# mct10/Speech-Vecalign

Measured on AMD Instinct MI355X. Metric: aligned doc-pairs/sec, higher is better.
Workload: dtype bf16; 1 GPU; synthetic 4096x4096 d=1024 bf16 embeddings, 4 overlap layers/side, 10 alignment types, band 14, coarse-to-fine (max_size_full_dp=300), 1024 doc-pairs per GPU per step; pipeline=1, N=4096, M=4096, d=1024, overlaps=4, parallelism=dp1 (pairs sharded, no collective)

## Files before the change

### include/svx.h

```cpp
#ifndef SVX_H
#define SVX_H

#include <stdint.h>

#ifdef __cplusplus
extern "C" {
#endif

typedef struct svx_ctx svx_ctx;

enum svx_dtype { SVX_F32 = 0, SVX_F16 = 1, SVX_BF16 = 2 };

enum svx_status {
    SVX_OK = 0,
    SVX_ERR_ARG = 1,
    SVX_ERR_OVERLAPS = 2,
    SVX_ERR_HIP = 3,
    SVX_ERR_TRACEBACK = 4,
    SVX_ERR_NOMEM = 5,
    SVX_ERR_EXTEND = 6,
    SVX_ERR_PATH = 7,
    SVX_ERR_BP = 8
};

#define SVX_MAX_LEVELS 16
#define SVX_MAX_TYPES 128
#define SVX_MAX_DIM 2048

int svx_create(int device_id, svx_ctx **out);
int svx_destroy(svx_ctx *ctx);
int svx_set_stream(svx_ctx *ctx, void *hip_stream);
int svx_synchronize(svx_ctx *ctx);
const char *svx_last_error(const svx_ctx *ctx);
const char *svx_version(void);
int64_t svx_scratch_bytes(const svx_ctx *ctx);


int svx_dense_costs(svx_ctx *ctx, const float *vecs0, int k0, int s0, const float *vecs1, int k1, int s1, int d,
                    const float *norm0, const float *norm1, int offset0, int offset1, float *costs);

int svx_dense_dp(svx_ctx *ctx, const float *cost, int s0, int s1, float pen, double *csum, int32_t *bp);

int svx_score_path(svx_ctx *ctx, const int32_t *xx, const int32_t *yy, int64_t n, const float *norm1,
                   const float *norm2, const float *vecs1, int rows1, const float *vecs2, int rows2, int d, float *out);

int svx_sparse_costs(svx_ctx *ctx, const float *vecs0, int k0, int xsize, const float *vecs1, int k1, int ysize,
                     int d, const float *norms0, const float *norms1, const int32_t *path, int A,
                     const int32_t *types_host, int T, int width_over2, float *costs, int32_t *b_offset);

int svx_sparse_dp(svx_ctx *ctx, const float *costs, const int32_t *b_offset_in, int A, int B,
                  const int32_t *types_host, int T, double del_penalty, int x_in_size, int y_in_size,
                  double *csum, int32_t *xp, int32_t *yp, int32_t *b_offset_out);


int svx_make_norm1(svx_ctx *ctx, float *vecs, int64_t rows, int d);

int svx_downsample(svx_ctx *ctx, const float *vecs, int k, int n, int d, float *half);

int svx_compute_norms(svx_ctx *ctx, const float *vecs0, int k0, int n0, const float *vecs1, int k1, int n1, int d,
                      const int32_t *idx, int samples_per_overlap, float *norms0);

int svx_del_penalty(svx_ctx *ctx, const float *scores, int64_t n, double frac, double *del_penalty);

int svx_dense_traceback(svx_ctx *ctx, const int32_t *bp, int s0, int s1, int32_t *align, int32_t *count);

int svx_sparse_traceback(svx_ctx *ctx, const double *csum, const int32_t *xp, const int32_t *yp,
                         const int32_t *b_offset_out, int a_out, int B, int xsize, int ysize, int32_t *align,
                         double *scores, int32_t *count);

int svx_search_path(svx_ctx *ctx, const int32_t *align, const int32_t *n_align, int upsample, int size0,
                    int size1, int32_t *path, int32_t *path_len);

int svx_gather_rows(svx_ctx *ctx, const void *table, int64_t n_rows, int d, int dtype, const int32_t *idx, int64_t n_out,
                    void *out);


int svx_mt19937_choice(uint32_t *key, int32_t *pos, int64_t n, int64_t size, int32_t *out);

int64_t svx_norm_index_count(int n, int m, int k0, int k1, int max_size_full_dp, int num_samps_for_norm, int have_norms0,
                             int have_norms1);
int64_t svx_knob_index_count(int n, int m, int max_size_full_dp, int costs_sample_size);

int svx_draw_indices(uint32_t *key, int32_t *pos, int n, int m, int k0, int k1, int max_size_full_dp, int costs_sample_size,
                     int num_samps_for_norm, int have_norms0, int have_norms1, int32_t *norm_idx, int32_t *knob_idx);

int svx_candidate_table(const char *seg_path, const char *cat_path, const char *ignore_path, int max_overlaps, int32_t *table,
                        int cap_lines, int32_t *n_lines, int64_t *n_candidates, char *err, int err_cap);

int64_t svx_format_alignments(const int32_t *rows, const double *scores, int64_t n, char *out, int64_t cap);


#define SVX_MARGIN_RATIO 0
#define SVX_MARGIN_DISTANCE 1
#define SVX_MARGIN_ABSOLUTE 2

int svx_unit_rows(svx_ctx *ctx, const void *rows, int dtype, int64_t n, int d, void *out, int out_dtype);

int svx_knn_mean_sim(svx_ctx *ctx, const void *queries, int q_dtype, int64_t n, const void *db, int db_dtype,
                     int64_t n_db, int d, int k, float *mean_sim);

int svx_knn_topk_merge(svx_ctx *ctx, const void *queries, int q_dtype, int64_t n, const void *db, int db_dtype,
                       int64_t n_db, int d, int k, float *topk, int first, float *mean_sim);

int svx_knn_search(svx_ctx *ctx, const void *queries, int q_dtype, int64_t n, const void *db, int db_dtype,
                   int64_t n_db, int d, int k, int64_t id_base, float *sims, int64_t *ids, int first);

int svx_knn_search_groups(svx_ctx *ctx, const void *queries, int q_dtype, const void *db, int db_dtype, int d, int k,
                          const int64_t *q_off, const int64_t *db_off, int n_groups, float *sims, int64_t *ids);

int svx_margin_scores(svx_ctx *ctx, const void *x, const void *y, int dtype, int64_t n, int d, const float *mean_xy,
                      const float *mean_yx, int margin, float *scores);


int svx_knn_list_means(svx_ctx *ctx, const float *sims, int64_t n, int k, float *mean);

int svx_margin_candidates(svx_ctx *ctx, const float *sims, const int64_t *ids, int64_t n, int k, const float *mean_q,
                          const float *mean_db, int64_t n_db, int64_t id_base, int margin, float *scores, int64_t *best_id,
                          float *best_score);

int64_t svx_mine_greedy(const int64_t *order, int64_t n_cand, const int64_t *src, const int64_t *tgt, int64_t n_src,
                        int64_t n_tgt, int64_t *out);


typedef struct svx_align_params {
    int32_t dtype;
    int32_t d;
    int32_t n_types;
    int32_t types[2 * SVX_MAX_TYPES];
    int32_t width_over2;
    int32_t max_size_full_dp;
    int32_t costs_sample_size;
    int32_t num_samps_for_norm;
    double del_percentile_frac;
    int32_t search_mode;
    int32_t reserved0;
} svx_align_params;

#define SVX_SEARCH_COARSE_TO_FINE 0
#define SVX_SEARCH_STRAIGHT 1

typedef struct svx_pair {
    const void *vecs0, *vecs1;
    int32_t n, m, k0, k1;
    const int32_t *norm_idx;
    const int32_t *knob_idx;
    const float *norms0, *norms1;
    int32_t *align;
    double *scores;
    int32_t *info;
    double *del_pen;
} svx_pair;

int svx_num_levels(int n, int m, int max_size_full_dp);
int64_t svx_knob_count(int n_l, int m_l, int costs_sample_size);

int svx_align_batch(svx_ctx *ctx, const svx_align_params *params, const svx_pair *pairs, int n_pairs);

int svx_alignment_rows(svx_ctx *ctx, int dtype, int d, const svx_pair *pairs, int n_pairs, double max_score, int64_t cap,
                       void *x_rows, void *y_rows, void *x_unit, void *y_unit, int unit_dtype, int32_t *src, int64_t *count);

#define SVX_CONCAT_MAX 8
typedef struct svx_frames { const int32_t *src, *tgt; } svx_frames;
typedef struct svx_concat_params {
    double  max_score;
    int32_t max_num_align;
    int32_t sample_rate;
    double  max_sil, max_dur;
    int32_t both_sides;
    int32_t pad;
    int64_t min_frames;
} svx_concat_params;
int svx_concat_rows(svx_ctx *ctx, int dtype, int d, const svx_pair *pairs, const svx_frames *frames, int n_pairs,
                    const svx_concat_params *params, int64_t cap, void *x_rows, void *y_rows, void *x_unit, void *y_unit,
                    int unit_dtype, int32_t *meta, int64_t *counts);

typedef struct svx_level_view {
    int32_t size0, size1, k0, k1;
    int32_t n_types, band;
    int32_t path_len, n_align;
    const float *n0, *n1;
    const double *del_penalty;
    const int32_t *searchpath;
    const float *a_b_costs;
    const int32_t *b_offset;
    const double *a_b_csum;
    const uint8_t *a_b_bp;
    const int32_t *a_b_xp, *a_b_yp;
    const int32_t *new_b_offset;
    const int32_t *alignments;
    const double *alignment_scores;
    const float *costs_1to1;
    const int32_t *x_y_tb_diag;
    const float *v0_l0, *v1_l0;
    const float *knob_scores;
    int32_t n_knob, reserved;
} svx_level_view;
int svx_debug_level(svx_ctx *ctx, int pair, int level, svx_level_view *out);
int svx_copy_to_host(svx_ctx *ctx, void *dst_host, const void *src_device, int64_t bytes);

int svx_set_profiling(svx_ctx *ctx, int on);
int svx_set_pipeline(svx_ctx *ctx, int on);
int svx_flush(svx_ctx *ctx);
double svx_stage_ms(svx_ctx *ctx, const char *stage);
int svx_stage_launches(svx_ctx *ctx, const char *stage);

#ifdef __cplusplus
}
#endif
#endif
```

### speech-vecalign_amd/csrc/svx_api.hip

```cpp
#include <stdarg.h>
#include <stdio.h>
#include <stdlib.h>
#include <string.h>

#include <chrono>
#include <functional>
#include <memory>
#include <type_traits>
#include <vector>

#include "svx_common.h"

static char g_err[512] = "";

int svx_fail(svx_ctx* ctx, int code, const char* fmt, ...) {
    char* dst = ctx ? ctx->err : g_err;
    va_list ap;
    va_start(ap, fmt);
    vsnprintf(dst, 512, fmt, ap);
    va_end(ap);
    return code;
}

static const char* kStageNames[] = {"pyr0",       "pyrN",     "pyr_aux",      "knob_scoresN", "knob",      "dense_costs",
                                    "dense_dp",   "path",     "band_costs0",  "band_costsN",  "band_dp0",  "band_dpN",
                                    "traceback",  "setup",    "total",        "host_plan",    "host_launch", "knob_sort", "knob_scores0", "pyr1", "tiles",
                                    "traceback0", "path0"};
enum {
    S_PYR0 = 0, S_PYRN, S_PYR_AUX, S_KNOB_SCORES, S_KNOB, S_DENSE_COSTS, S_DENSE_DP, S_PATH, S_BAND_COSTS0, S_BAND_COSTSN,
    S_BAND_DP0, S_BAND_DPN, S_TRACEBACK, S_SETUP, S_TOTAL, S_HOST_PLAN, S_HOST_LAUNCH, S_KNOB_SORT, S_KNOB_SCORES0, S_PYR1, S_TILES,
    S_TRACEBACK0, S_PATH0, S_COUNT
};

struct StageRec {
    int stage;
    hipEvent_t a, b;
};

struct BatchParams {
    SvxTypes tfinal, t11;
    int W, B, dtype, d, nsamp, n_types;
    double frac;
    bool straight, tiles, packable;
};

struct HalfState {
    char* arena = nullptr;
    size_t arena_bytes = 0;
    SvxPairDev* pinned = nullptr;
    size_t pinned_cap = 0;
    std::vector<SvxPairDev> host;
    SvxPairDev* dpairs = nullptr;
    int n_pairs = 0;
    int maxL = 0, max_ksum = 0, max_kn = 0, max_ds0 = 0, max_ds1 = 0, max_n0 = 0, max_tnd = 0;
    int max_nblk[SVX_MAX_LEVELS] = {0}, max_A[SVX_MAX_LEVELS] = {0};
    bool any_L0 = false;
    size_t o_tickets = 0;
    size_t o_planes = 0, b_planes = 0;
    double b_pyr[SVX_MAX_LEVELS] = {0}, b_bc[SVX_MAX_LEVELS] = {0}, b_knobN = 0, b_knob0 = 0, dense_cells = 0;
    BatchParams bp;
    bool chain_pending = false;
    bool chain_done_valid = false;
    hipEvent_t front_done = nullptr, chain_done = nullptr, upload_done = nullptr;
    bool upload_valid = false;
};

struct svx_ctx_ext : svx_ctx {
    double ms[S_COUNT];
    int launches[S_COUNT];
    std::vector<StageRec> recs;
    std::vector<StageRec> pending;
    double acc_ms[S_COUNT];
    long long acc_launches[S_COUNT];
    int pipeline;
    HalfState half[2];
    int last_split;
    hipStream_t chain;
    bool chain_ready;
    std::vector<hipEvent_t> ev_pool;
    size_t ev_next;
    hipStream_t side;
    hipStream_t helper;
    hipEvent_t side_fork, side_join;
    bool side_ready;
    int last_ntypes, last_band;
};

static inline svx_ctx_ext* X(svx_ctx* c) { return static_cast<svx_ctx_ext*>(c); }

struct StageScope {
    svx_ctx_ext* c;
    StageRec r;
    bool on;
    StageScope(svx_ctx* ctx, int stage) : c(X(ctx)), on(ctx->profiling != 0) {
        r.stage = stage;
        if (on) {
            (void)hipEventCreate(&r.a);
            (void)hipEventCreate(&r.b);
            (void)hipEventRecord(r.a, c->stream);
        }
    }
    ~StageScope() {
        if (on) {
            (void)hipEventRecord(r.b, c->stream);
            c->recs.push_back(r);
        }
        c->launches[r.stage]++;
    }
};

static void drop_pending(svx_ctx_ext* c) {
    for (auto& r : c->pending) { (void)hipEventDestroy(r.a); (void)hipEventDestroy(r.b); }
    c->pending.clear();
}

extern "C" {

const char* svx_version(void) { return "svx 0.1 (gfx950)"; }

int svx_create(int device_id, svx_ctx** out) {
    if (!out) return svx_fail(nullptr, SVX_ERR_ARG, "svx_create: out is NULL");
    int ndev = 0;
    hipError_t e = hipGetDeviceCount(&ndev);
    if (e != hipSuccess || ndev <= 0)
        return svx_fail(nullptr, SVX_ERR_HIP, "svx_create: no HIP device (%s)", hipGetErrorString(e));
    if (device_id < 0 || device_id >= ndev) return svx_fail(nullptr, SVX_ERR_ARG, "svx_create: device %d of %d", device_id, ndev);
    e = hipSetDevice(device_id);
    if (e != hipSuccess) return svx_fail(nullptr, SVX_ERR_HIP, "hipSetDevice: %s", hipGetErrorString(e));
    svx_ctx_ext* c = new svx_ctx_ext();
    c->device = device_id;
    c->stream = nullptr;
    c->arena = nullptr;
    c->arena_bytes = 0;
    c->arena_used = 0;
    c->err[0] = 0;
    c->profiling = 0;
    c->rows_buf = nullptr;
    c->rows_bytes = 0;
    c->rows_turn = 0;
    for (int i = 0; i < 2; i++) { c->rows_pin[i] = nullptr; c->rows_pin_cap[i] = 0; c->rows_up[i] = nullptr; c->rows_up_valid[i] = 0; }
    for (int i = 0; i < S_COUNT; i++) { c->ms[i] = -1.0; c->launches[i] = 0; }
    c->pipeline = 0;
    c->last_split = 0;
    c->chain = nullptr;
    c->chain_ready = false;
    c->ev_next = 0;
    c->last_ntypes = 0;
    c->last_band = 0;
    c->side_ready = false;
    *out = c;
    return SVX_OK;
}

int svx_destroy(svx_ctx* ctx) {
    if (!ctx) return SVX_OK;
    svx_ctx_ext* c = X(ctx);
    (void)hipSetDevice(ctx->device);
    (void)svx_flush(ctx);
    (void)hipStreamSynchronize(ctx->stream);
    if (c->chain_ready) (void)hipStreamSynchronize(c->chain);
    if (ctx->arena) (void)hipFree(ctx->arena);
    svxl_alignrows_release(ctx);
    drop_pending(c);
    for (auto& r : c->recs) { (void)hipEventDestroy(r.a); (void)hipEventDestroy(r.b); }
    if (c->side_ready) {
        (void)hipStreamSynchronize(c->side);
        (void)hipStreamDestroy(c->side);
        (void)hipStreamSynchronize(c->helper);
        (void)hipStreamDestroy(c->helper);
        (void)hipEventDestroy(c->side_fork);
        (void)hipEventDestroy(c->side_join);
    }
    if (c->chain_ready) (void)hipStreamDestroy(c->chain);
    for (auto e : c->ev_pool) (void)hipEventDestroy(e);
    for (int h = 0; h < 2; h++) {
        HalfState& H = c->half[h];
        if (H.arena) (void)hipFree(H.arena);
        if (H.pinned) (void)hipHostFree(H.pinned);
        if (H.front_done) (void)hipEventDestroy(H.front_done);
        if (H.chain_done) (void)hipEventDestroy(H.chain_done);
        if (H.upload_done) (void)hipEventDestroy(H.upload_done);
    }
    delete c;
    return SVX_OK;
}

int svx_set_stream(svx_ctx* ctx, void* hip_stream) {
    if (!ctx) return SVX_ERR_ARG;
    ctx->stream = reinterpret_cast<hipStream_t>(hip_stream);
    return SVX_OK;
}

int svx_synchronize(svx_ctx* ctx) {
    if (!ctx) return SVX_ERR_ARG;
    int rc = svx_flush(ctx);
    if (rc) return rc;
    SVX_HIP(ctx, hipStreamSynchronize(ctx->stream));
    return SVX_OK;
}

const char* svx_last_error(const svx_ctx* ctx) { return ctx ? ctx->err : g_err; }

int64_t svx_scratch_bytes(const svx_ctx* ctx) {
    if (!ctx) return 0;
    const svx_ctx_ext* c = static_cast<const svx_ctx_ext*>(ctx);
    return (int64_t)(ctx->arena_bytes + c->half[0].arena_bytes + c->half[1].arena_bytes + ctx->rows_bytes);
}

int svx_set_pipeline(svx_ctx* ctx, int on) {
    if (!ctx || on < 0 || on > 1) return SVX_ERR_ARG;
    if (X(ctx)->pipeline != on) {
        int rc = svx_flush(ctx);
        if (rc) return rc;
    }
    X(ctx)->pipeline = on;
    return SVX_OK;
}

static void fold_pending(svx_ctx_ext* c) {
    if (c->pending.empty()) return;
    (void)svx_flush(c);
    (void)hipStreamSynchronize(c->stream);
    if (c->side_ready) { (void)hipStreamSynchronize(c->side); (void)hipStreamSynchronize(c->helper); }
    for (auto& r : c->pending) {
        float ms = 0.f;
        if (hipEventElapsedTime(&ms, r.a, r.b) == hipSuccess) { c->acc_ms[r.stage] += ms; }
        (void)hipEventDestroy(r.a);
        (void)hipEventDestroy(r.b);
    }
    c->pending.clear();
}

int svx_set_profiling(svx_ctx* ctx, int on) {
    if (!ctx) return SVX_ERR_ARG;
    svx_ctx_ext* c = X(ctx);
    drop_pending(c);
    ctx->profiling = on;
    if (on == 2)
        for (int i = 0; i < S_COUNT; i++) { c->acc_ms[i] = 0.0; c->acc_launches[i] = 0; }
    return SVX_OK;
}

static int stage_index(const char* name) {
    for (int i = 0; i < S_COUNT; i++)
        if (strcmp(name, kStageNames[i]) == 0) return i;
    return -1;
}

double svx_stage_ms(svx_ctx* ctx, const char* stage) {
    if (!ctx || !stage) return -1.0;
    int i = stage_index(stage);
    if (i < 0) return -1.0;
    if (ctx->profiling == 2) {
        fold_pending(X(ctx));
        return X(ctx)->acc_ms[i];
    }
    return X(ctx)->ms[i];
}

int svx_stage_launches(svx_ctx* ctx, const char* stage) {
    if (!ctx || !stage) return -1;
    int i = stage_index(stage);
    if (i < 0) return -1;
    if (ctx->profiling == 2) return (int)X(ctx)->acc_launches[i];
    return X(ctx)->launches[i];
}

}

static int arena_reserve(svx_ctx* ctx, size_t bytes) {
    if (bytes <= ctx->arena_bytes) return SVX_OK;
    SVX_HIP(ctx, hipStreamSynchronize(ctx->stream));
    if (ctx->arena) SVX_HIP(ctx, hipFree(ctx->arena));
    ctx->arena = nullptr;
    ctx->arena_bytes = 0;
    size_t want = bytes + bytes / 16 + (1 << 20);
    hipError_t e = hipMalloc(&ctx->arena, want);
    if (e != hipSuccess) return svx_fail(ctx, SVX_ERR_NOMEM, "scratch arena: hipMalloc(%zu) failed: %s", want, hipGetErrorString(e));
    ctx->arena_bytes = want;
    return SVX_OK;
}

struct Bump;
template <class T>
static inline void set_off(T*& p, Bump& b, size_t bytes);

struct Bump {
    size_t off = 0;
    size_t take(size_t bytes) {
        size_t o = off;
        off += (bytes + 255) & ~(size_t)255;
        return o;
    }
};

template <class T>
static inline void set_off(T*& p, Bump& b, size_t bytes) {
    p = reinterpret_cast<T*>(b.take(bytes) + 1);
}

static int make_types(svx_ctx* ctx, const int32_t* types, int T, SvxTypes* out) {
    if (T < 0 || T > SVX_MAX_TYPES) return svx_fail(ctx, SVX_ERR_ARG, "%d alignment types (max %d)", T, SVX_MAX_TYPES);
    out->n = T;
    out->maxstep = 1;
    for (int t = 0; t < T; t++) {
        int x = types[2 * t], y = types[2 * t + 1];
        if (x < 1 || y < 1 || x > 100 || y > 100) return svx_fail(ctx, SVX_ERR_ARG, "alignment type (%d,%d): sizes must be >= 1", x, y);
        out->x[t] = (int8_t)x;
        out->y[t] = (int8_t)y;
        if (x + y > out->maxstep) out->maxstep = x + y;
    }
    out->x[T] = 0; out->y[T] = 1;
    out->x[T + 1] = 1; out->y[T + 1] = 0;
    return SVX_OK;
}

static int check_dim(svx_ctx* ctx, int d) {
    if (d <= 0 || d % 8 != 0 || d > SVX_MAX_DIM)
        return svx_fail(ctx, SVX_ERR_ARG, "embedding dimension %d: must be a positive multiple of 8, at most %d", d, SVX_MAX_DIM);
    return SVX_OK;
}

#define NEED(ctx, cond, ...) \
    do { if (!(cond)) return svx_fail(ctx, SVX_ERR_ARG, __VA_ARGS__); } while (0)

extern "C" {

int svx_dense_costs(svx_ctx* ctx, const float* vecs0, int k0, int s0, const float* vecs1, int k1, int s1, int d,
                    const float* norm0, const float* norm1, int offset0, int offset1, float* costs) {
    NEED(ctx, ctx && vecs0 && vecs1 && norm0 && norm1 && costs, "svx_dense_costs: null argument");
    NEED(ctx, k0 > offset0 && k1 > offset1 && offset0 >= 0 && offset1 >= 0, "svx_dense_costs: offsets (%d,%d) outside %d/%d layers", offset0, offset1, k0, k1);
    int rc = check_dim(ctx, d);
    if (rc) return rc;
    return svxl_dense_costs(ctx, vecs0 + (size_t)offset0 * s0 * d, s0, vecs1 + (size_t)offset1 * s1 * d, s1, d,
                            norm0 + (size_t)offset0 * s0, norm1 + (size_t)offset1 * s1, offset0 + 1, offset1 + 1, costs);
}

int svx_dense_dp(svx_ctx* ctx, const float* cost, int s0, int s1, float pen, double* csum, int32_t* bp) {
    NEED(ctx, ctx && bp && (cost || s0 == 0 || s1 == 0), "svx_dense_dp: null argument");
    NEED(ctx, s0 >= 0 && s1 >= 0, "svx_dense_dp: negative size");
    return svxl_dense_dp(ctx, cost, s0, s1, pen, csum, bp);
}

int svx_score_path(svx_ctx* ctx, const int32_t* xx, const int32_t* yy, int64_t n, const float* norm1, const float* norm2,
                   const float* vecs1, int rows1, const float* vecs2, int rows2, int d, float* out) {
    NEED(ctx, ctx && xx && yy && norm1 && norm2 && vecs1 && vecs2 && out, "svx_score_path: null argument");
    NEED(ctx, rows1 > 0 && rows2 > 0, "svx_score_path: empty vecs");
    int rc = check_dim(ctx, d);
    if (rc) return rc;
    return svxl_score_path(ctx, xx, yy, n, norm1, norm2, vecs1, rows1, vecs2, rows2, d, out);
}

int svx_sparse_costs(svx_ctx* ctx, const float* vecs0, int k0, int xsize, const float* vecs1, int k1, int ysize, int d,
                     const float* norms0, const float* norms1, const int32_t* path, int A, const int32_t* types_host, int T,
                     int width_over2, float* costs, int32_t* b_offset) {
    NEED(ctx, ctx && vecs0 && vecs1 && norms0 && norms1 && path && b_offset && (costs || T == 0), "svx_sparse_costs: null argument");
    NEED(ctx, width_over2 >= 1 && A >= 0, "svx_sparse_costs: bad width/path length");
    int rc = check_dim(ctx, d);
    if (rc) return rc;
    SvxTypes ty;
    rc = make_types(ctx, types_host, T, &ty);
    if (rc) return rc;
    int mx = 0, my = 0;
    for (int t = 0; t < T; t++) { if (ty.x[t] > mx) mx = ty.x[t]; if (ty.y[t] > my) my = ty.y[t]; }
    if (mx > k0) return svx_fail(ctx, SVX_ERR_OVERLAPS, "%d x overlaps requrested (via alignment_types), but vecs0 only has %d", mx, k0);
    if (my > k1) return svx_fail(ctx, SVX_ERR_OVERLAPS, "%d y overlaps requrested (via alignment_types), but vecs1 only has %d", my, k1);
    rc = arena_reserve(ctx, 256);
    if (rc) return rc;
    int* status = reinterpret_cast<int*>(ctx->arena);
    SVX_HIP(ctx, hipMemsetAsync(status, 0, sizeof(int), ctx->stream));
    rc = svxl_band_costs(ctx, vecs0, k0, xsize, vecs1, k1, ysize, d, SVX_F32, nullptr, nullptr, norms0, norms1, path, A, ty,
                         width_over2, costs, b_offset, status);
    if (rc) return rc;
    int hs = 0;
    SVX_HIP(ctx, hipMemcpyAsync(&hs, status, sizeof(int), hipMemcpyDeviceToHost, ctx->stream));
    SVX_HIP(ctx, hipStreamSynchronize(ctx->stream));
    if (hs != 0) return svx_fail(ctx, hs, "search path is not a unit-step lattice path starting at (0,0)");
    return SVX_OK;
}

int svx_sparse_dp(svx_ctx* ctx, const float* costs, const int32_t* b_offset_in, int A, int B, const int32_t* types_host,
                  int T, double del_penalty, int x_in_size, int y_in_size, double* csum, int32_t* xp, int32_t* yp,
                  int32_t* b_offset_out) {
    NEED(ctx, ctx && b_offset_in && csum && xp && yp && b_offset_out && (costs || T == 0), "svx_sparse_dp: null argument");
    NEED(ctx, A >= 1 && B >= 1, "svx_sparse_dp: empty cost band");
    SvxTypes ty;
    int rc = make_types(ctx, types_host, T, &ty);
    if (rc) return rc;
    return svxl_sparse_dp(ctx, costs, b_offset_in, A, B, ty, del_penalty, x_in_size, y_in_size, csum, xp, yp, b_offset_out);
}

int svx_make_norm1(svx_ctx* ctx, float* vecs, int64_t rows, int d) {
    NEED(ctx, ctx && (vecs || rows == 0), "svx_make_norm1: null argument");
    int rc = check_dim(ctx, d);
    if (rc) return rc;
    return svxl_make_norm1(ctx, vecs, rows, d);
}

int svx_downsample(svx_ctx* ctx, const float* vecs, int k, int n, int d, float* half) {
    NEED(ctx, ctx && vecs && (half || n < 2), "svx_downsample: null argument");
    int rc = check_dim(ctx, d);
    if (rc) return rc;
    const int h = n / 2;
    if (h <= 0 || k <= 0) return SVX_OK;
    const int nblk = (h + SVX_PYR_SLOTS - 1) / SVX_PYR_SLOTS;
    Bump b;
    size_t o_part = b.take((size_t)k * nblk * d * sizeof(float));
    size_t o_mean = b.take((size_t)k * d * sizeof(float));
    rc = arena_reserve(ctx, b.off);
    if (rc) return rc;
    float* part = reinterpret_cast<float*>(ctx->arena + o_part);
    float* mean = reinterpret_cast<float*>(ctx->arena + o_mean);
    if ((rc = svxl_pairsum(ctx, vecs, k, n, d, half, part, nblk))) return rc;
    if ((rc = svxl_colmean_plain(ctx, part, k, nblk, d, h, mean))) return rc;
    return svxl_sub_mean(ctx, half, k, h, d, mean);
}

int svx_compute_norms(svx_ctx* ctx, const float* vecs0, int k0, int n0, const float* vecs1, int k1, int n1, int d,
                      const int32_t* idx, int samples_per_overlap, float* norms0) {
    NEED(ctx, ctx && vecs0 && vecs1 && idx && norms0, "svx_compute_norms: null argument");
    NEED(ctx, n1 > 0 && samples_per_overlap > 0 && k1 > 0, "svx_compute_norms: nothing to sample");
    int rc = check_dim(ctx, d);
    if (rc) return rc;
    rc = arena_reserve(ctx, (size_t)d * sizeof(float) + 256);
    if (rc) return rc;
    float* rbar = reinterpret_cast<float*>(ctx->arena);
    if ((rc = svxl_sample_mean_plain(ctx, vecs1, k1, n1, d, idx, samples_per_overlap, rbar))) return rc;
    return svxl_norms_from_rbar(ctx, vecs0, (int64_t)k0 * n0, d, rbar, norms0);
}

int svx_del_penalty(svx_ctx* ctx, const float* scores, int64_t n, double frac, double* del_penalty) {
    NEED(ctx, ctx && scores && del_penalty && n > 0, "svx_del_penalty: null/empty argument");
    return svxl_del_penalty(ctx, scores, n, frac, del_penalty);
}

int svx_dense_traceback(svx_ctx* ctx, const int32_t* bp, int s0, int s1, int32_t* align, int32_t* count) {
    NEED(ctx, ctx && bp && align && count, "svx_dense_traceback: null argument");
    return svxl_dense_traceback(ctx, bp, s0, s1, align, count);
}

int svx_sparse_traceback(svx_ctx* ctx, const double* csum, const int32_t* xp, const int32_t* yp, const int32_t* b_offset_out,
                         int a_out, int B, int xsize, int ysize, int32_t* align, double* scores, int32_t* count) {
    NEED(ctx, ctx && csum && xp && yp && b_offset_out && align && scores && count, "svx_sparse_traceback: null argument");
    return svxl_sparse_traceback(ctx, csum, xp, yp, b_offset_out, a_out, B, xsize, ysize, align, scores, count);
}

int svx_search_path(svx_ctx* ctx, const int32_t* align, const int32_t* n_align, int upsample, int size0, int size1,
                    int32_t* path, int32_t* path_len) {
    NEED(ctx, ctx && align && n_align && path && path_len, "svx_search_path: null argument");
    return svxl_search_path(ctx, align, n_align, upsample, size0, size1, path, size0 + size1 + 4, path_len);
}

int svx_gather_rows(svx_ctx* ctx, const void* table, int64_t n_rows, int d, int dtype, const int32_t* idx, int64_t n_out, void* out) {
    NEED(ctx, ctx && table && idx && out, "svx_gather_rows: null argument");
    NEED(ctx, dtype == SVX_F32 || dtype == SVX_F16 || dtype == SVX_BF16, "svx_gather_rows: unknown dtype %d", dtype);
    int rc = check_dim(ctx, d);
    if (rc) return rc;
    return svxl_gather_rows(ctx, table, n_rows, d * (dtype == SVX_F32 ? 4 : 2), dtype, idx, n_out, out);
}

}

__global__ void k_init_batch(const SvxPairDev* pairs) {
    const SvxPairDev& P = pairs[blockIdx.x];
    if (threadIdx.x != 0) return;
    *P.status = 0;
    for (int l = 0; l <= P.L; l++) {
        if (P.lev[l].n_align) *P.lev[l].n_align = 0;
        if (P.lev[l].path_len) *P.lev[l].path_len = 0;
    }
    if (P.straight) {
        int* r = P.lev[0].align;
        r[0] = 0; r[1] = P.lev[0].n[0]; r[2] = 0; r[3] = P.lev[0].n[1];
        *P.lev[0].n_align = 1;
    }
}

static inline int ceil_div(int a, int b) { return (a + b - 1) / b; }

extern "C" int svx_copy_to_host(svx_ctx* ctx, void* dst_host, const void* src_device, int64_t bytes) {
    NEED(ctx, ctx && (bytes == 0 || (dst_host && src_device)) && bytes >= 0, "svx_copy_to_host: bad argument");
    if (bytes == 0) return SVX_OK;
    SVX_HIP(ctx, hipSetDevice(ctx->device));
    SVX_HIP(ctx, hipMemcpyAsync(dst_host, src_device, (size_t)bytes, hipMemcpyDeviceToHost, ctx->stream));
    SVX_HIP(ctx, hipStreamSynchronize(ctx->stream));
    return SVX_OK;
}

extern "C" int svx_debug_level(svx_ctx* ctx, int pair, int level, svx_level_view* out) {
    NEED(ctx, ctx && out, "svx_debug_level: null argument");
    svx_ctx_ext* cx = X(ctx);
    const int total = cx->half[0].n_pairs + (cx->last_split > 0 ? cx->half[1].n_pairs : 0);
    NEED(ctx, pair >= 0 && pair < total, "svx_debug_level: pair %d of the last batch (%d pairs)", pair, total);
    const bool second = cx->last_split > 0 && pair >= cx->last_split;
    const SvxPairDev& P = second ? cx->half[1].host[pair - cx->last_split] : cx->half[0].host[pair];
    NEED(ctx, level >= 0 && level <= P.L, "svx_debug_level: level %d (the pair has %d)", level, P.L + 1);
    const SvxLevel& Lv = P.lev[level];
    memset(out, 0, sizeof(*out));
    out->size0 = Lv.n[0]; out->size1 = Lv.n[1];
    out->k0 = P.K[0]; out->k1 = P.K[1];
    out->n_types = level == 0 ? cx->last_ntypes : 1;
    out->band = cx->last_band;
    out->n0 = Lv.nrm[0]; out->n1 = Lv.nrm[1];
    out->del_penalty = Lv.pen;
    SVX_HIP(ctx, hipSetDevice(ctx->device));
    int rc = svx_synchronize(ctx);
    if (rc) return rc;
    if (Lv.n_align) SVX_HIP(ctx, hipMemcpy(&out->n_align, Lv.n_align, sizeof(int), hipMemcpyDeviceToHost));
    out->alignments = Lv.align;
    const bool refined = (level < P.L) || (P.L == 0);
    if (refined) {
        SVX_HIP(ctx, hipMemcpy(&out->path_len, Lv.path_len, sizeof(int), hipMemcpyDeviceToHost));
        out->searchpath = Lv.path;
        out->a_b_costs = Lv.costs;
        out->b_offset = Lv.boff;
        out->a_b_csum = Lv.csum;
        out->a_b_bp = Lv.bpk;
        out->a_b_xp = Lv.xp;
        out->a_b_yp = Lv.yp;
        out->new_b_offset = Lv.boff_out;
        out->alignment_scores = Lv.scores;
    }
    if (level == P.L && !P.straight) {
        out->costs_1to1 = P.dcost;
        out->x_y_tb_diag = P.dbp;
    }
    out->knob_scores = Lv.kscore;
    out->n_knob = Lv.kn;
    if (level >= 1) {
        out->v0_l0 = Lv.P[0];
        out->v1_l0 = Lv.P[1];
    }
    return SVX_OK;
}

static int plan_half(svx_ctx* ctx, HalfState& H, const BatchParams& bp, const svx_align_params* prm, const svx_pair* pairs, int n_pairs) {
    const int d = bp.d;
    const size_t esz = bp.dtype == SVX_F32 ? 4 : 2;
    const SvxTypes& tfinal = bp.tfinal;
    const int B = bp.B;
    const bool straight = bp.straight, tiles = bp.tiles, packable = bp.packable;
    int mx = 0, my = 0;
    for (int t = 0; t < tfinal.n; t++) { if (tfinal.x[t] > mx) mx = tfinal.x[t]; if (tfinal.y[t] > my) my = tfinal.y[t]; }
    std::vector<SvxPairDev>& host = H.host;
    host.assign(n_pairs, SvxPairDev());
    H.n_pairs = n_pairs;
    H.bp = bp;
    H.maxL = H.max_ksum = H.max_kn = H.max_ds0 = H.max_ds1 = H.max_n0 = H.max_tnd = 0;
    H.any_L0 = false;
    H.o_tickets = 0;
    H.o_planes = H.b_planes = 0;
    H.b_knobN = H.b_knob0 = H.dense_cells = 0;
    for (int l = 0; l < SVX_MAX_LEVELS; l++) { H.max_nblk[l] = H.max_A[l] = 0; H.b_pyr[l] = H.b_bc[l] = 0; }
    Bump bump;
    const size_t o_desc = bump.take((size_t)n_pairs * sizeof(SvxPairDev));
#define OFF(ptr_field, bytes) set_off(ptr_field, bump, bytes)
    for (int p = 0; p < n_pairs; p++) {
        const svx_pair& in = pairs[p];
        SvxPairDev& P = host[p];
        memset(&P, 0, sizeof(P));
        NEED(ctx, in.vecs0 && in.vecs1 && in.align && in.scores && in.info && in.knob_idx, "pair %d: null pointer", p);
        NEED(ctx, in.n >= 1 && in.m >= 1 && in.k0 >= 1 && in.k1 >= 1, "pair %d: empty document or no overlap layers", p);
        if (mx > in.k0) return svx_fail(ctx, SVX_ERR_OVERLAPS, "%d x overlaps requrested (via alignment_types), but vecs0 only has %d", mx, in.k0);
        if (my > in.k1) return svx_fail(ctx, SVX_ERR_OVERLAPS, "%d y overlaps requrested (via alignment_types), but vecs1 only has %d", my, in.k1);
        const int L = straight ? 0 : svx_num_levels(in.n, in.m, prm->max_size_full_dp);
        P.straight = straight ? 1 : 0;
        NEED(ctx, L < SVX_MAX_LEVELS, "pair %d: %d pyramid levels (max %d)", p, L + 1, SVX_MAX_LEVELS);
        P.v[0] = in.vecs0; P.v[1] = in.vecs1;
        P.K[0] = in.k0; P.K[1] = in.k1;
        P.L = L; P.d = d;
        P.norm_override[0] = in.norms0 != nullptr;
        P.norm_override[1] = in.norms1 != nullptr;
        P.status = in.info + 1;
        if (L > H.maxL) H.maxL = L;
        if (in.n > H.max_n0) H.max_n0 = in.n;
        if (L == 0) H.any_L0 = true;
        if (in.k0 + in.k1 > H.max_ksum) H.max_ksum = in.k0 + in.k1;
        const int S_from[2] = {in.k0 > 0 ? ceil_div(prm->num_samps_for_norm, in.k0) : 0,
                               in.k1 > 0 ? ceil_div(prm->num_samps_for_norm, in.k1) : 0};
        const int32_t* nidx = in.norm_idx;
        const int32_t* kidx = in.knob_idx;
        for (int l = 0; l <= L; l++) {
            SvxLevel& Lv = P.lev[l];
            const int K[2] = {in.k0, in.k1};
            for (int s = 0; s < 2; s++) {
                Lv.n[s] = (s == 0 ? in.n : in.m) >> l;
                Lv.nblk[s] = ceil_div((Lv.n[s] + 1) / 2, SVX_PYR_SLOTS);
                if (Lv.nblk[s] > H.max_nblk[l]) H.max_nblk[l] = Lv.nblk[s];
            }
            for (int s = 1; s >= 0; s--) {
                const bool skip = (l == 0) && P.norm_override[1 - s];
                Lv.S[s] = skip ? 0 : S_from[s];
                Lv.sidx[s] = nullptr;
                if (Lv.S[s] > 0) {
                    NEED(ctx, nidx != nullptr, "pair %d: norm_idx is NULL", p);
                    Lv.sidx[s] = nidx;
                    nidx += (size_t)K[s] * Lv.S[s];
                }
            }
            for (int s = 0; s < 2; s++) {
                if (l >= 1) {
                    Lv.npart[s] = P.lev[l - 1].nblk[s];
                    OFF(Lv.P[s], (size_t)(l == 1 ? 1 : K[s]) * Lv.n[s] * d * sizeof(float));
                    OFF(Lv.part[s], (size_t)K[s] * Lv.npart[s] * d * sizeof(float));
                    OFF(Lv.mean[s], (size_t)K[s] * d * sizeof(float));
                } else {
                    OFF(Lv.inv[s], (size_t)K[s] * Lv.n[s] * sizeof(float));
                }
                OFF(Lv.rbar[s], (size_t)d * sizeof(float));
                if (l == 0 && P.norm_override[s]) Lv.nrm[s] = const_cast<float*>(s == 0 ? in.norms0 : in.norms1);
                else OFF(Lv.nrm[s], (size_t)K[s] * Lv.n[s] * sizeof(float));
            }
            const int64_t kn = svx_knob_count(Lv.n[0], Lv.n[1], prm->costs_sample_size);
            Lv.kn = (int)kn;
            Lv.kx = kidx;
            Lv.ky = kidx + kn;
            kidx += 2 * kn;
            if (Lv.kn > H.max_kn) H.max_kn = Lv.kn;
            OFF(Lv.kscore, (size_t)kn * sizeof(float));
            OFF(Lv.korder, (size_t)kn * sizeof(int));
            OFF(Lv.kys, (size_t)kn * sizeof(int));
            OFF(Lv.kstart, (size_t)(Lv.n[0] + 1) * sizeof(int));
            if (in.del_pen) Lv.pen = in.del_pen + l;
            else OFF(Lv.pen, sizeof(double));
            const bool refined = (l < L) || (L == 0);
            const int rows_cap = Lv.n[0] + Lv.n[1] + 2;
            if (refined) {
                const int cap = Lv.n[0] + Lv.n[1] + 4;
                const int T = (l == 0) ? tfinal.n : 1;
                Lv.path_cap = cap;
                if (cap > H.max_A[l]) H.max_A[l] = cap;
                OFF(Lv.path, (size_t)cap * 2 * sizeof(int));
                OFF(Lv.path_len, sizeof(int));
                OFF(Lv.cstart, (size_t)(cap / 16 + 3) * sizeof(int));
                OFF(Lv.nchunks, sizeof(int));
                if (!tiles) OFF(Lv.costs, (size_t)(T > 0 ? T : 1) * cap * B * sizeof(float));
                OFF(Lv.boff, (size_t)cap * sizeof(int));
                OFF(Lv.csum, (size_t)(cap + 2) * B * sizeof(double));
                if (packable) {
                    OFF(Lv.bpk, (size_t)(cap + 2) * B);
                } else {
                    OFF(Lv.xp, (size_t)(cap + 2) * B * sizeof(int));
                    OFF(Lv.yp, (size_t)(cap + 2) * B * sizeof(int));
                }
                OFF(Lv.boff_out, (size_t)(cap + 2) * sizeof(int));
            }
            if (l == 0) {
                Lv.align = in.align;
                Lv.scores = in.scores;
                Lv.n_align = in.info;
            } else {
                OFF(Lv.align, (size_t)rows_cap * 4 * sizeof(int));
                OFF(Lv.scores, (size_t)rows_cap * sizeof(double));
                OFF(Lv.n_align, sizeof(int));
            }
            const double krows = (double)K[0] * Lv.n[0] + (double)K[1] * Lv.n[1], rows = (double)Lv.n[0] + Lv.n[1];
            if (l == 0) {
                H.b_pyr[0] += krows * d * esz;
                H.b_bc[0] += krows * d * esz;
                H.b_knob0 += (double)kn * d * esz;
            } else {
                if (l == 1) H.b_pyr[1] += ((double)K[0] * in.n + (double)K[1] * in.m) * d * esz + rows * d * 4.0;
                else H.b_pyr[l] += (krows + rows) * d * 4.0;
                H.b_pyr[l - 1] += l >= 2 ? krows * d * 4.0 : 0.0;
                if (l < L) { H.b_bc[l] += rows * d * 4.0; H.b_knobN += (double)kn * d * 4.0; }
            }
        }
        const SvxLevel& top = P.lev[L];
        if (!straight) {
            if (top.n[0] > H.max_ds0) H.max_ds0 = top.n[0];
            if (top.n[1] > H.max_ds1) H.max_ds1 = top.n[1];
            H.dense_cells += (double)top.n[0] * top.n[1];
            OFF(P.dcost, (size_t)top.n[0] * top.n[1] * sizeof(float));
            OFF(P.ddot, (size_t)top.n[0] * top.n[1] * sizeof(float));
            OFF(P.dbp, (size_t)(top.n[0] + top.n[1] + 1) * (top.n[0] + 1) * sizeof(int));
        }
        if (tiles) {
            const long long TI = in.n / 32 + 1, TJ = in.m / 32 + 1;
            P.t_nd = (int)(TI + TJ - 1);
            long long tcap = (long long)P.t_nd * ((B + 64) / 32 + 2);
            if (tcap > TI * TJ) tcap = TI * TJ;
            NEED(ctx, tcap < (1ll << 30), "pair %d: too many tiles", p);
            P.t_cap = (int)tcap;
            OFF(P.t_lo, (size_t)P.t_nd * sizeof(int));
            OFF(P.t_cnt, (size_t)P.t_nd * sizeof(int));
            OFF(P.t_pref, (size_t)(P.t_nd + 1) * sizeof(int));
            OFF(P.t_flag, (size_t)P.t_cap * sizeof(int));
        }
    }
#undef OFF
    for (int p = 0; p < n_pairs; p++)
        if (host[p].t_nd > H.max_tnd) H.max_tnd = host[p].t_nd;
    if (tiles) {
        H.o_tickets = bump.take(((size_t)(H.max_tnd + 2) * n_pairs + 2) * sizeof(int));
        H.b_planes = svxl_band_tiles_scratch(tfinal);
        if (H.b_planes) H.o_planes = bump.take(H.b_planes);
    }
    if (bump.off > H.arena_bytes) {
        SVX_HIP(ctx, hipDeviceSynchronize());
        if (H.arena) SVX_HIP(ctx, hipFree(H.arena));
        H.arena = nullptr;
        H.arena_bytes = 0;
        const size_t want = bump.off + bump.off / 16 + (1 << 20);
        hipError_t e = hipMalloc(&H.arena, want);
        if (e != hipSuccess) return svx_fail(ctx, SVX_ERR_NOMEM, "scratch arena: hipMalloc(%zu) failed: %s", want, hipGetErrorString(e));
        H.arena_bytes = want;
    }
    const size_t desc_bytes = (size_t)n_pairs * sizeof(SvxPairDev);
    if (desc_bytes > H.pinned_cap) {
        SVX_HIP(ctx, hipDeviceSynchronize());
        if (H.pinned) SVX_HIP(ctx, hipHostFree(H.pinned));
        H.pinned = nullptr;
        H.pinned_cap = 0;
        SVX_HIP(ctx, hipHostMalloc(reinterpret_cast<void**>(&H.pinned), desc_bytes + desc_bytes / 8, hipHostMallocDefault));
        H.pinned_cap = desc_bytes + desc_bytes / 8;
    }
    char* base = H.arena;
    const char* ulo = reinterpret_cast<const char*>(1);
    const char* uhi = reinterpret_cast<const char*>(bump.off + 1);
    auto patch = [&](auto& ptr) {
        const char* v = reinterpret_cast<const char*>(ptr);
        if (v >= ulo && v < uhi) ptr = reinterpret_cast<typename std::remove_reference<decltype(ptr)>::type>(base + (v - ulo));
    };
    for (int p = 0; p < n_pairs; p++) {
        SvxPairDev& P = host[p];
        const svx_pair& in = pairs[p];
        for (int l = 0; l <= P.L; l++) {
            SvxLevel& Lv = P.lev[l];
            for (int s = 0; s < 2; s++) {
                patch(Lv.P[s]); patch(Lv.part[s]); patch(Lv.mean[s]); patch(Lv.rbar[s]); patch(Lv.inv[s]);
                if (!(l == 0 && P.norm_override[s])) patch(Lv.nrm[s]);
            }
            patch(Lv.kscore); patch(Lv.korder); patch(Lv.kys); patch(Lv.kstart);
            if (!in.del_pen) patch(Lv.pen);
            patch(Lv.path); patch(Lv.path_len); patch(Lv.cstart); patch(Lv.nchunks); patch(Lv.costs); patch(Lv.boff); patch(Lv.csum); patch(Lv.xp); patch(Lv.yp); patch(Lv.bpk);
            patch(Lv.boff_out);
            if (l > 0) { patch(Lv.align); patch(Lv.scores); patch(Lv.n_align); }
        }
        patch(P.dcost);
        patch(P.ddot);
        patch(P.dbp);
        patch(P.t_lo); patch(P.t_cnt); patch(P.t_pref); patch(P.t_flag);
    }
    H.dpairs = reinterpret_cast<SvxPairDev*>(base + o_desc);
    return SVX_OK;
}

struct Op {
    double us;
    int stage;
    std::function<int()> fn;
};

static int run_op(svx_ctx* ctx, const Op& op, hipStream_t st) {
    hipStream_t keep = ctx->stream;
    ctx->stream = st;
    int rc;
    if (op.stage < 0) {
        rc = op.fn();
    } else {
        StageScope sc(ctx, op.stage);
        rc = op.fn();
    }
    ctx->stream = keep;
    return rc;
}

static int next_event(svx_ctx* ctx, hipEvent_t* out) {
    svx_ctx_ext* cx = X(ctx);
    if (cx->ev_pool.size() < 256) {
        hipEvent_t e;
        SVX_HIP(ctx, hipEventCreateWithFlags(&e, hipEventDisableTiming));
        cx->ev_pool.push_back(e);
        *out = e;
        return SVX_OK;
    }
    *out = cx->ev_pool[cx->ev_next++ % cx->ev_pool.size()];
    return SVX_OK;
}

static void front_ops(svx_ctx* ctx, HalfState& H, std::vector<Op>& ops, int split) {
    svx_ctx_ext* cx = X(ctx);
    HalfState* h = &H;
    const BatchParams& bp = H.bp;
    const int np = H.n_pairs, d = bp.d, dtype = bp.dtype;
    const double waves = (double)((np + 1023) / 1024);
    const int parts = (split > 1 && np >= 16 * split) ? split : 1;
    struct Evs { hipEvent_t pass[SVX_MAX_LEVELS][8]; };
    auto evs = std::make_shared<Evs>();
    ops.push_back({0.0, -1, [=]() -> int {
        SVX_HIP(ctx, hipEventRecord(cx->side_fork, ctx->stream));
        SVX_HIP(ctx, hipStreamWaitEvent(cx->side, cx->side_fork, 0));
        SVX_HIP(ctx, hipStreamWaitEvent(cx->helper, cx->side_fork, 0));
        return SVX_OK;
    }});
    auto sort_op = [=]() -> int {
        hipStream_t main_stream = ctx->stream;
        static const bool inline_sort = getenv("SVX_SORT_INLINE") != nullptr;
        if (parts > 1 && !inline_sort) SVX_HIP(ctx, hipStreamWaitEvent(cx->side, evs->pass[0][parts - 1], 0));
        ctx->stream = inline_sort ? main_stream : cx->side;
        int rc;
        {
            StageScope sc(ctx, S_KNOB_SORT);
            rc = svxl_knob_scores(ctx, h->dpairs, np, h->maxL, h->max_kn, h->max_n0, dtype, d, 0);
        }
        ctx->stream = main_stream;
        if (rc) return rc;
        SVX_HIP(ctx, hipEventRecord(cx->side_join, inline_sort ? main_stream : cx->side));
        return SVX_OK;
    };
    if (parts == 1) ops.push_back({0.0, -1, sort_op});
    for (int l = 0; l <= H.maxL; l++) {
        for (int q = 0; q < parts; q++) {
            const int lo = (int)((long long)np * q / parts), hi = (int)((long long)np * (q + 1) / parts);
            const double aux_us = (l == 0 ? 700.0 * waves : 250.0) / parts;
            if (parts == 1) {
                ops.push_back({aux_us, S_PYR_AUX, [=]() { return svxl_pyramid_level(ctx, h->dpairs, np, l, dtype, d, h->max_nblk[l], h->max_ksum, 0); }});
                ops.push_back({H.b_pyr[l] / (l == 0 ? 4.9e6 : 5.3e6), l == 0 ? S_PYR0 : (l == 1 ? S_PYR1 : S_PYRN),
                               [=]() { return svxl_pyramid_level(ctx, h->dpairs, np, l, dtype, d, h->max_nblk[l], h->max_ksum, 1); }});
                continue;
            }
            ops.push_back({H.b_pyr[l] / (l == 0 ? 4.9e6 : 5.3e6) / parts, l == 0 ? S_PYR0 : (l == 1 ? S_PYR1 : S_PYRN), [=]() -> int {
                hipStream_t main_stream = ctx->stream;
                int rc;
                if (l == 0 && q == 0) {
                    StageScope sc(ctx, S_PYR_AUX);
                    if ((rc = svxl_pyramid_level(ctx, h->dpairs + lo, hi - lo, l, dtype, d, h->max_nblk[l], h->max_ksum, 0))) return rc;
                } else {
                    if (l > 0) SVX_HIP(ctx, hipStreamWaitEvent(cx->helper, evs->pass[l - 1][q], 0));
                    ctx->stream = cx->helper;
                    {
                        StageScope sc(ctx, S_PYR_AUX);
                        rc = svxl_pyramid_level(ctx, h->dpairs + lo, hi - lo, l, dtype, d, h->max_nblk[l], h->max_ksum, 0);
                    }
                    ctx->stream = main_stream;
                    if (rc) return rc;
                    hipEvent_t aux_done;
                    if ((rc = next_event(ctx, &aux_done))) return rc;
                    SVX_HIP(ctx, hipEventRecord(aux_done, cx->helper));
                    SVX_HIP(ctx, hipStreamWaitEvent(main_stream, aux_done, 0));
                }
                if ((rc = svxl_pyramid_level(ctx, h->dpairs + lo, hi - lo, l, dtype, d, h->max_nblk[l], h->max_ksum, 1))) return rc;
                if ((rc = next_event(ctx, &evs->pass[l][q]))) return rc;
                SVX_HIP(ctx, hipEventRecord(evs->pass[l][q], main_stream));
                return SVX_OK;
            }});
        }
        if (parts > 1 && l == 0) ops.push_back({0.0, -1, sort_op});
    }
    if (!bp.straight) {
        ops.push_back({H.dense_cells * 2.7e-5, S_DENSE_COSTS, [=]() -> int {
            int rc = svxl_dense_costs_batch(ctx, h->dpairs, np, h->max_ds0, h->max_ds1, dtype, d);
            if (rc) return rc;
            return svxl_knob_from_dots(ctx, h->dpairs, np, h->max_kn);
        }});
    }
    if (H.maxL >= 1) {
        ops.push_back({H.b_knobN / 16.5e6, S_KNOB_SCORES, [=]() -> int {
            SVX_HIP(ctx, hipStreamWaitEvent(ctx->stream, cx->side_join, 0));
            return svxl_knob_scores(ctx, h->dpairs, np, h->maxL, h->max_kn, h->max_n0, dtype, d, 1);
        }});
    }
    ops.push_back({H.b_knob0 / 8.5e6, S_KNOB_SCORES0, [=]() -> int {
        SVX_HIP(ctx, hipStreamWaitEvent(ctx->stream, cx->side_join, 0));
        return svxl_knob_scores(ctx, h->dpairs, np, h->maxL, h->max_kn, h->max_n0, dtype, d, 2);
    }});
}

struct Seg {
    std::vector<Op> lb;
    bool has_s = false;
    Op s;
};

static void chain_segs(svx_ctx* ctx, HalfState& H, std::vector<Seg>& segs) {
    HalfState* h = &H;
    const BatchParams bp = H.bp;
    const int np = H.n_pairs, d = bp.d, dtype = bp.dtype, W = bp.W, B = bp.B;
    const double waves = (double)((np + 1023) / 1024);
    Seg cur;
    cur.lb.push_back({(np * (H.maxL + 1) * 0.21 < 300.0 ? 300.0 : np * (H.maxL + 1) * 0.21), S_KNOB,
                      [=]() { return svxl_del_penalty_batch(ctx, h->dpairs, np, h->maxL + 1, bp.frac); }});
    if (!bp.straight)
        cur.lb.push_back({(H.max_ds0 + H.max_ds1) * 1.7 * waves, S_DENSE_DP, [=]() { return svxl_dense_stage_batch(ctx, h->dpairs, np, h->max_ds0); }});
    const int first_depth = H.maxL > 0 ? H.maxL - 1 : 0;
    for (int depth = first_depth; depth >= 0; depth--) {
        const SvxTypes ty = depth == 0 ? bp.tfinal : bp.t11;
        int lim2 = 0, tamax2 = 0;
        const bool v2 = !bp.tiles && svxl_band2_limits(ty, W, depth, dtype, d, &lim2, &tamax2);
        const int maxA = H.max_A[depth];
        const int src_rows = (H.maxL > 0 && !H.any_L0) ? maxA / 2 + 8 : maxA;
        cur.lb.push_back({maxA * 0.08 * waves + 60.0, depth == 0 ? S_PATH0 : S_PATH, [=]() {
            return svxl_search_path_batch(ctx, h->dpairs, np, depth, maxA, src_rows, v2 ? lim2 : SVX_BC_ROWS - SVX_BC_TB,
                                          bp.tiles ? 0 : (v2 ? tamax2 : SVX_BC_TAMAX));
        }});
        cur.has_s = true;
        if (bp.tiles) {
            cur.s = {1.0e4, S_TILES, [=]() {
                int* tk = reinterpret_cast<int*>(h->arena + h->o_tickets);
                float* planes = h->b_planes ? reinterpret_cast<float*>(h->arena + h->o_planes) : nullptr;
                return svxl_band_tiles_batch(ctx, h->dpairs, np, ty, W, dtype, h->max_tnd, tk, tk + (size_t)h->max_tnd * np + 1, planes);
            }};
        } else {
            cur.s = {H.b_bc[depth] / 4.0e6, depth == 0 ? S_BAND_COSTS0 : S_BAND_COSTSN, [=]() {
                return v2 ? svxl_band_costs2_batch(ctx, h->dpairs, np, depth, maxA, ty, W, dtype, d)
                          : svxl_band_costs_batch(ctx, h->dpairs, np, depth, maxA, ty, W, dtype, d);
            }};
        }
        segs.push_back(cur);
        cur = Seg();
        if (!bp.tiles)
            cur.lb.push_back({maxA * (0.21 + 0.054 * (ty.n > 1 ? ty.n : 0)) * waves, depth == 0 ? S_BAND_DP0 : S_BAND_DPN,
                              [=]() { return svxl_sparse_dp_batch(ctx, h->dpairs, np, depth, ty, B); }});
        cur.lb.push_back({maxA * 0.27 * waves, depth == 0 ? S_TRACEBACK0 : S_TRACEBACK, [=]() { return svxl_sparse_traceback_batch(ctx, h->dpairs, np, depth, B, maxA, bp.packable ? 1 : 0); }});
    }
    segs.push_back(cur);
}

static int ensure_streams(svx_ctx* ctx) {
    svx_ctx_ext* cx = X(ctx);
    if (!cx->side_ready) {
        int prio_lo = 0, prio_hi = 0;
        SVX_HIP(ctx, hipDeviceGetStreamPriorityRange(&prio_lo, &prio_hi));
        SVX_HIP(ctx, hipStreamCreateWithPriority(&cx->side, hipStreamNonBlocking, prio_lo));
        SVX_HIP(ctx, hipStreamCreateWithPriority(&cx->helper, hipStreamNonBlocking, prio_hi));
        SVX_HIP(ctx, hipEventCreateWithFlags(&cx->side_fork, hipEventDisableTiming));
        SVX_HIP(ctx, hipEventCreateWithFlags(&cx->side_join, hipEventDisableTiming));
        cx->side_ready = true;
    }
    if (!cx->chain_ready) {
        int prio_lo = 0, prio_hi = 0;
        SVX_HIP(ctx, hipDeviceGetStreamPriorityRange(&prio_lo, &prio_hi));
        SVX_HIP(ctx, hipStreamCreateWithPriority(&cx->chain, hipStreamNonBlocking, prio_hi));
        cx->chain_ready = true;
    }
    for (int h = 0; h < 2; h++) {
        if (!cx->half[h].front_done) SVX_HIP(ctx, hipEventCreateWithFlags(&cx->half[h].front_done, hipEventDisableTiming));
        if (!cx->half[h].chain_done) SVX_HIP(ctx, hipEventCreateWithFlags(&cx->half[h].chain_done, hipEventDisableTiming));
        if (!cx->half[h].upload_done) SVX_HIP(ctx, hipEventCreateWithFlags(&cx->half[h].upload_done, hipEventDisableTiming));
    }
    return SVX_OK;
}

static int run_interleaved(svx_ctx* ctx, HalfState* front, HalfState* chain, bool beside) {
    svx_ctx_ext* cx = X(ctx);
    hipStream_t A = ctx->stream, Bst = beside ? cx->chain : ctx->stream;
    std::vector<Op> fops;
    std::vector<Seg> segs;
    if (front) {
        if (front->chain_done_valid) SVX_HIP(ctx, hipStreamWaitEvent(A, front->chain_done, 0));
        {
            StageScope sc(ctx, S_SETUP);
            if (front->upload_valid) SVX_HIP(ctx, hipEventSynchronize(front->upload_done));
            memcpy(front->pinned, front->host.data(), (size_t)front->n_pairs * sizeof(SvxPairDev));
            SVX_HIP(ctx, hipMemcpyAsync(front->dpairs, front->pinned, (size_t)front->n_pairs * sizeof(SvxPairDev), hipMemcpyHostToDevice, A));
            SVX_HIP(ctx, hipEventRecord(front->upload_done, A));
            front->upload_valid = true;
            hipLaunchKernelGGL(k_init_batch, dim3(front->n_pairs), dim3(64), 0, A, front->dpairs);
            SVX_LAUNCH_CHECK(ctx, "k_init_batch");
            if (front->bp.nsamp == 0) {
                for (int p = 0; p < front->n_pairs; p++)
                    for (int l = 0; l <= front->host[p].L; l++)
                        for (int s = 0; s < 2; s++)
                            SVX_HIP(ctx, hipMemsetAsync(front->host[p].lev[l].rbar[s], 0, (size_t)front->bp.d * sizeof(float), A));
            }
        }
        static const int split_env = [] { const char* e = getenv("SVX_PIPE_SPLIT"); const int v = e ? atoi(e) : 2; return v >= 1 && v <= 8 ? v : 2; }();
        front_ops(ctx, *front, fops, beside ? split_env : 1);
    }
    if (chain) chain_segs(ctx, *chain, segs);
    int rc;
    size_t fi = 0;
    if (chain && beside) SVX_HIP(ctx, hipStreamWaitEvent(Bst, chain->front_done, 0));
    for (size_t g = 0; g < segs.size(); g++) {
        double need = 0.0;
        for (const Op& op : segs[g].lb) {
            if ((rc = run_op(ctx, op, Bst))) return rc;
            need += op.us;
        }
        hipEvent_t lb_done = nullptr;
        if (beside) {
            if ((rc = next_event(ctx, &lb_done))) return rc;
            SVX_HIP(ctx, hipEventRecord(lb_done, Bst));
        }
        if (!segs[g].has_s) break;
        double acc = 0.0;
        need = need * 1.25 + 50.0;
        while (beside && fi < fops.size() && acc < need) {
            if ((rc = run_op(ctx, fops[fi], A))) return rc;
            acc += fops[fi].us;
            fi++;
        }
        if (beside) SVX_HIP(ctx, hipStreamWaitEvent(A, lb_done, 0));
        if ((rc = run_op(ctx, segs[g].s, A))) return rc;
        if (beside) {
            hipEvent_t s_done;
            if ((rc = next_event(ctx, &s_done))) return rc;
            SVX_HIP(ctx, hipEventRecord(s_done, A));
            SVX_HIP(ctx, hipStreamWaitEvent(Bst, s_done, 0));
        }
    }
    for (; fi < fops.size(); fi++)
        if ((rc = run_op(ctx, fops[fi], A))) return rc;
    if (front) {
        SVX_HIP(ctx, hipEventRecord(front->front_done, A));
        front->chain_pending = true;
    }
    if (chain) {
        SVX_HIP(ctx, hipEventRecord(chain->chain_done, Bst));
        chain->chain_done_valid = true;
        chain->chain_pending = false;
    }
    return SVX_OK;
}

extern "C" int svx_flush(svx_ctx* ctx) {
    if (!ctx) return SVX_ERR_ARG;
    svx_ctx_ext* cx = X(ctx);
    bool any = false;
    for (int h = 0; h < 2; h++) any = any || cx->half[h].chain_pending || cx->half[h].chain_done_valid;
    if (!any) return SVX_OK;
    SVX_HIP(ctx, hipSetDevice(ctx->device));
    int rc;
    for (int h = 0; h < 2; h++)
        if (cx->half[h].chain_pending && (rc = run_interleaved(ctx, nullptr, &cx->half[h], true))) return rc;
    for (int h = 0; h < 2; h++)
        if (cx->half[h].chain_done_valid) SVX_HIP(ctx, hipStreamWaitEvent(ctx->stream, cx->half[h].chain_done, 0));
    return SVX_OK;
}

extern "C" int svx_align_batch(svx_ctx* ctx, const svx_align_params* prm, const svx_pair* pairs, int n_pairs) {
    NEED(ctx, ctx && prm && (pairs || n_pairs == 0), "svx_align_batch: null argument");
    if (n_pairs <= 0) return SVX_OK;
    const auto t_enter = std::chrono::steady_clock::now();
    svx_ctx_ext* cx = X(ctx);
    SVX_HIP(ctx, hipSetDevice(ctx->device));
    int rc = check_dim(ctx, prm->d);
    if (rc) return rc;
    BatchParams bp;
    bp.d = prm->d;
    bp.dtype = prm->dtype;
    NEED(ctx, bp.dtype == SVX_F32 || bp.dtype == SVX_F16 || bp.dtype == SVX_BF16, "svx_align_batch: unknown dtype %d", bp.dtype);
    NEED(ctx, prm->max_size_full_dp >= 1, "svx_align_batch: max_size_full_dp must be >= 1");
    NEED(ctx, prm->costs_sample_size >= 1, "svx_align_batch: costs_sample_size must be >= 1");
    NEED(ctx, prm->num_samps_for_norm >= 0, "svx_align_batch: num_samps_for_norm must be >= 0");
    if ((rc = make_types(ctx, prm->types, prm->n_types, &bp.tfinal))) return rc;
    const int32_t one_one[2] = {1, 1};
    make_types(ctx, one_one, 1, &bp.t11);
    bp.W = prm->width_over2 < 3 ? 3 : prm->width_over2;
    bp.B = 2 * bp.W;
    bp.nsamp = prm->num_samps_for_norm;
    bp.frac = prm->del_percentile_frac;
    bp.n_types = bp.tfinal.n;
    int mx = 0, my = 0;
    for (int t = 0; t < bp.tfinal.n; t++) { if (bp.tfinal.x[t] > mx) mx = bp.tfinal.x[t]; if (bp.tfinal.y[t] > my) my = bp.tfinal.y[t]; }
    bp.packable = mx <= 15 && my <= 15;
    NEED(ctx, prm->search_mode == SVX_SEARCH_COARSE_TO_FINE || prm->search_mode == SVX_SEARCH_STRAIGHT, "svx_align_batch: unknown search_mode %d", prm->search_mode);
    bp.straight = prm->search_mode == SVX_SEARCH_STRAIGHT;
    bp.tiles = bp.straight && bp.B > 64;
    if (bp.tiles) NEED(ctx, bp.tfinal.n >= 1 && svxl_band_tiles_shape(bp.tfinal) >= 0, "wide straight band: no tile shape takes these %d alignment types", bp.tfinal.n);
    if ((rc = ensure_streams(ctx))) return rc;
    for (int i = 0; i < S_COUNT; i++) { cx->ms[i] = 0.0; cx->launches[i] = 0; }
    for (auto& r : cx->recs) { (void)hipEventDestroy(r.a); (void)hipEventDestroy(r.b); }
    cx->recs.clear();
    const bool piped = cx->pipeline != 0 && !bp.tiles && n_pairs >= 2;
    double plan_ms = 0.0;
    {
        StageScope total(ctx, S_TOTAL);
        if (!piped) {
            if ((rc = svx_flush(ctx))) return rc;
            HalfState& H = cx->half[0];
            if ((rc = plan_half(ctx, H, bp, prm, pairs, n_pairs))) return rc;
            cx->last_split = 0;
            plan_ms = std::chrono::duration<double, std::milli>(std::chrono::steady_clock::now() - t_enter).count();
            if ((rc = run_interleaved(ctx, &H, nullptr, false))) return rc;
            if ((rc = run_interleaved(ctx, nullptr, &H, false))) return rc;
            H.chain_done_valid = false;
        } else {
            const int n0 = (n_pairs + 1) / 2;
            HalfState &H0 = cx->half[0], &H1 = cx->half[1];
            if (H0.chain_pending && (rc = run_interleaved(ctx, nullptr, &H0, true))) return rc;
            auto t0 = std::chrono::steady_clock::now();
            if ((rc = plan_half(ctx, H0, bp, prm, pairs, n0))) return rc;
            plan_ms += std::chrono::duration<double, std::milli>(std::chrono::steady_clock::now() - t0).count();
            if ((rc = run_interleaved(ctx, &H0, H1.chain_pending ? &H1 : nullptr, true))) return rc;
            t0 = std::chrono::steady_clock::now();
            if ((rc = plan_half(ctx, H1, bp, prm, pairs + n0, n_pairs - n0))) return rc;
            plan_ms += std::chrono::duration<double, std::milli>(std::chrono::steady_clock::now() - t0).count();
            cx->last_split = n0;
            if ((rc = run_interleaved(ctx, &H1, &H0, true))) return rc;
        }
    }
    cx->last_ntypes = bp.tfinal.n;
    cx->last_band = bp.B;
    const auto t_done = std::chrono::steady_clock::now();
    cx->ms[S_HOST_PLAN] = plan_ms;
    cx->ms[S_HOST_LAUNCH] = std::chrono::duration<double, std::milli>(t_done - t_enter).count() - plan_ms;
    if (ctx->profiling == 2) {
        for (auto& r : cx->recs) cx->pending.push_back(r);
        cx->recs.clear();
        for (int i = 0; i < S_COUNT; i++) cx->acc_launches[i] += cx->launches[i];
        cx->acc_ms[S_HOST_PLAN] += cx->ms[S_HOST_PLAN];
        cx->acc_ms[S_HOST_LAUNCH] += cx->ms[S_HOST_LAUNCH];
    } else if (ctx->profiling) {
        if ((rc = svx_synchronize(ctx))) return rc;
        if (cx->side_ready) { SVX_HIP(ctx, hipStreamSynchronize(cx->side)); SVX_HIP(ctx, hipStreamSynchronize(cx->helper)); }
        for (auto& r : cx->recs) {
            float ms = 0.f;
            if (hipEventElapsedTime(&ms, r.a, r.b) == hipSuccess) cx->ms[r.stage] += ms;
            (void)hipEventDestroy(r.a);
            (void)hipEventDestroy(r.b);
        }
        cx->recs.clear();
    }
    return SVX_OK;
}
```

### speech-vecalign_amd/csrc/svx_common.h

```cpp
#pragma once
#include <hip/hip_runtime.h>
#include <stdint.h>
#include <stddef.h>
#include "../../include/svx.h"

#define SVX_WAVE 64

#ifndef SVX_PYR_SLOTS
#define SVX_PYR_SLOTS 32
#endif
#define SVX_BC_TA 32
#define SVX_BC_TAMAX 64
#define SVX_BC_TB 16
#define SVX_BC_ROWS 48

struct ElemF32 {
    using storage = float;
    static constexpr int VEC = 4;
    static constexpr int DT = SVX_F32;
};
struct ElemF16 {
    using storage = uint16_t;
    static constexpr int VEC = 8;
    static constexpr int DT = SVX_F16;
};
struct ElemBF16 {
    using storage = uint16_t;
    static constexpr int VEC = 8;
    static constexpr int DT = SVX_BF16;
};

__device__ __forceinline__ float bf16_to_f32(uint16_t h) { return __uint_as_float(((uint32_t)h) << 16); }
__device__ __forceinline__ float f16_to_f32(uint16_t h) { return (float)__builtin_bit_cast(_Float16, h); }

#define SVX_GLOBAL(T) __attribute__((address_space(1))) T
typedef uint32_t svx_u32x4 __attribute__((ext_vector_type(4)));
typedef float svx_f32x4 __attribute__((ext_vector_type(4)));
template <typename T>
__device__ __forceinline__ T gld(const T* p) { return *(const SVX_GLOBAL(T)*)p; }
template <typename T>
__device__ __forceinline__ void gst(T* p, T v) { *(SVX_GLOBAL(T)*)p = v; }
__device__ __forceinline__ uint4 gld16(const void* p) {
    const svx_u32x4 v = *(const SVX_GLOBAL(svx_u32x4)*)p;
    return make_uint4(v.x, v.y, v.z, v.w);
}
__device__ __forceinline__ uint4 gld16_nt(const void* p) {
    const svx_u32x4 v = __builtin_nontemporal_load((const SVX_GLOBAL(svx_u32x4)*)p);
    return make_uint4(v.x, v.y, v.z, v.w);
}
__device__ __forceinline__ void gst16(void* p, uint32_t a, uint32_t b, uint32_t c, uint32_t d) {
    const svx_u32x4 v = {a, b, c, d};
    *(SVX_GLOBAL(svx_u32x4)*)p = v;
}
__device__ __forceinline__ float4 gldf4(const float* p) {
    const svx_f32x4 v = *(const SVX_GLOBAL(svx_f32x4)*)p;
    return make_float4(v.x, v.y, v.z, v.w);
}
__device__ __forceinline__ void gstf4(float* p, float a, float b, float c, float d) {
    const svx_f32x4 v = {a, b, c, d};
    *(SVX_GLOBAL(svx_f32x4)*)p = v;
}
__device__ __forceinline__ void gstf4_nt(float* p, float a, float b, float c, float d) {
    const svx_f32x4 v = {a, b, c, d};
    __builtin_nontemporal_store(v, (SVX_GLOBAL(svx_f32x4)*)p);
}

template <typename E>
__device__ __forceinline__ void decode_piece(const uint4& v, float* out);
template <>
__device__ __forceinline__ void decode_piece<ElemF32>(const uint4& v, float* out) {
    out[0] = __uint_as_float(v.x); out[1] = __uint_as_float(v.y); out[2] = __uint_as_float(v.z); out[3] = __uint_as_float(v.w);
}
template <>
__device__ __forceinline__ void decode_piece<ElemF16>(const uint4& v, float* out) {
    const uint32_t w[4] = {v.x, v.y, v.z, v.w};
#pragma unroll
    for (int i = 0; i < 4; i++) {
        out[2 * i] = f16_to_f32((uint16_t)(w[i] & 0xffffu));
        out[2 * i + 1] = f16_to_f32((uint16_t)(w[i] >> 16));
    }
}
template <>
__device__ __forceinline__ void decode_piece<ElemBF16>(const uint4& v, float* out) {
    const uint32_t w[4] = {v.x, v.y, v.z, v.w};
#pragma unroll
    for (int i = 0; i < 4; i++) {
        out[2 * i] = __uint_as_float(w[i] << 16);
        out[2 * i + 1] = __uint_as_float(w[i] & 0xffff0000u);
    }
}
template <typename E>
__device__ __forceinline__ void gload_piece(const typename E::storage* p, float* out) {
    decode_piece<E>(gld16(p), out);
}

template <typename E>
__device__ __forceinline__ void load_piece(const typename E::storage* p, float* out);
template <>
__device__ __forceinline__ void load_piece<ElemF32>(const float* p, float* out) {
    float4 v = *reinterpret_cast<const float4*>(p);
    out[0] = v.x; out[1] = v.y; out[2] = v.z; out[3] = v.w;
}
template <>
__device__ __forceinline__ void load_piece<ElemF16>(const uint16_t* p, float* out) {
    uint4 v = *reinterpret_cast<const uint4*>(p);
    uint32_t w[4] = {v.x, v.y, v.z, v.w};
#pragma unroll
    for (int i = 0; i < 4; i++) {
        out[2 * i] = f16_to_f32((uint16_t)(w[i] & 0xffffu));
        out[2 * i + 1] = f16_to_f32((uint16_t)(w[i] >> 16));
    }
}
template <>
__device__ __forceinline__ void load_piece<ElemBF16>(const uint16_t* p, float* out) {
    uint4 v = *reinterpret_cast<const uint4*>(p);
    uint32_t w[4] = {v.x, v.y, v.z, v.w};
#pragma unroll
    for (int i = 0; i < 4; i++) {
        out[2 * i] = __uint_as_float(w[i] << 16);
        out[2 * i + 1] = __uint_as_float(w[i] & 0xffff0000u);
    }
}

__device__ __forceinline__ unsigned xchg16_u32(unsigned v, int lane) {
    auto r = __builtin_amdgcn_permlane16_swap(v, v, false, false);
    return ((lane >> 4) & 1) ? r[0] : r[1];
}
__device__ __forceinline__ unsigned xchg32_u32(unsigned v, int lane) {
    auto r = __builtin_amdgcn_permlane32_swap(v, v, false, false);
    return (lane & 32) ? r[0] : r[1];
}
#define SVX_DPP_F32(v, ctrl) __builtin_bit_cast(float, __builtin_amdgcn_update_dpp(0, __builtin_bit_cast(int, (v)), (ctrl), 0xf, 0xf, false))

__device__ __forceinline__ float wave_sum(float v) {
    const int lane = threadIdx.x & 63;
    v += SVX_DPP_F32(v, 0xB1);
    v += SVX_DPP_F32(v, 0x4E);
    v += SVX_DPP_F32(v, 0x141);
    v += SVX_DPP_F32(v, 0x140);
    v += __uint_as_float(xchg16_u32(__float_as_uint(v), lane));
    v += __uint_as_float(xchg32_u32(__float_as_uint(v), lane));
    return v;
}
__device__ __forceinline__ float wave_max(float v) {
    const int lane = threadIdx.x & 63;
    v = fmaxf(v, SVX_DPP_F32(v, 0xB1));
    v = fmaxf(v, SVX_DPP_F32(v, 0x4E));
    v = fmaxf(v, SVX_DPP_F32(v, 0x141));
    v = fmaxf(v, SVX_DPP_F32(v, 0x140));
    v = fmaxf(v, __uint_as_float(xchg16_u32(__float_as_uint(v), lane)));
    v = fmaxf(v, __uint_as_float(xchg32_u32(__float_as_uint(v), lane)));
    return v;
}

struct SvxLevel {
    int n[2];
    int nblk[2];
    int npart[2];
    int S[2];
    float* P[2];
    float* part[2];
    float* mean[2];
    float* rbar[2];
    float* inv[2];
    float* nrm[2];
    const int* sidx[2];
    const int* kx;
    const int* ky;
    int kn;
    int path_cap;
    float* kscore;
    int* korder;
    int* kys;
    int* kstart;
    double* pen;
    int* path;
    int* path_len;
    int* cstart;
    int* nchunks;
    float* costs;
    int* boff;
    double* csum;
    int* xp;
    int* yp;
    unsigned char* bpk;
    int* boff_out;
    int* align;
    int* n_align;
    double* scores;
};

struct SvxPairDev {
    const void* v[2];
    int K[2];
    int L;
    int d;
    int norm_override[2];
    float* dcost;
    float* ddot;
    int* dbp;
    int* status;
    int straight;
    int t_nd, t_cap;
    int* t_lo;
    int* t_cnt;
    int* t_pref;
    int* t_flag;
    SvxLevel lev[SVX_MAX_LEVELS];
};

struct SvxTypes {
    int n;
    int maxstep;
    int8_t x[SVX_MAX_TYPES + 2];
    int8_t y[SVX_MAX_TYPES + 2];
};

struct svx_ctx {
    int device;
    hipStream_t stream;
    char* arena;
    size_t arena_bytes;
    size_t arena_used;
    char err[512];
    int profiling;
    char* rows_buf;
    size_t rows_bytes;
    char* rows_pin[2];
    size_t rows_pin_cap[2];
    hipEvent_t rows_up[2];
    int rows_up_valid[2];
    int rows_turn;
};

int svx_fail(svx_ctx* ctx, int code, const char* fmt, ...);
#define SVX_HIP(ctx, call)                                                                     \
    do {                                                                                       \
        hipError_t e_ = (call);                                                                \
        if (e_ != hipSuccess) return svx_fail(ctx, SVX_ERR_HIP, "%s: %s", #call, hipGetErrorString(e_)); \
    } while (0)
#define SVX_LAUNCH_CHECK(ctx, name)                                                            \
    do {                                                                                       \
        hipError_t e_ = hipGetLastError();                                                     \
        if (e_ != hipSuccess) return svx_fail(ctx, SVX_ERR_HIP, "launch %s: %s", name, hipGetErrorString(e_)); \
    } while (0)

void svxl_alignrows_release(svx_ctx*);
int svxl_make_norm1(svx_ctx*, float* vecs, int64_t rows, int d);
int svxl_pairsum(svx_ctx*, const float* vecs, int k, int n, int d, float* half, float* part, int nblk);
int svxl_colmean_plain(svx_ctx*, const float* part, int k, int nblk, int d, int count, float* mean);
int svxl_sub_mean(svx_ctx*, float* half, int k, int h, int d, const float* mean);
int svxl_sample_mean_plain(svx_ctx*, const float* vecs, int k, int n, int d, const int* idx, int S, float* rbar);
int svxl_norms_from_rbar(svx_ctx*, const float* vecs, int64_t rows, int d, const float* rbar, float* norms);
int svxl_gather_rows(svx_ctx*, const void* table, long long n_rows, int row_bytes, int dtype, const int* idx, long long n_out, void* out);
int svxl_pyramid_level(svx_ctx*, const SvxPairDev* pairs, int n_pairs, int level, int dtype, int d, int max_nblk,
                       int max_ksum, int part);
int svxl_score_path(svx_ctx*, const int* xx, const int* yy, int64_t n, const float* n1, const float* n2,
                    const float* v1, int rows1, const float* v2, int rows2, int d, float* out);
int svxl_knob_scores(svx_ctx*, const SvxPairDev* pairs, int n_pairs, int max_levels, int max_kn, int max_n0, int dtype, int d,
                     int part);
int svxl_dense_costs(svx_ctx*, const float* v0, int s0, const float* v1, int s1, int d, const float* n0,
                     const float* n1, int mul0, int mul1, float* costs);
int svxl_dense_costs_batch(svx_ctx*, const SvxPairDev* pairs, int n_pairs, int max_s0, int max_s1, int dtype, int d);
int svxl_knob_from_dots(svx_ctx*, const SvxPairDev* pairs, int n_pairs, int max_kn);
int svxl_band_costs(svx_ctx*, const void* v0, int k0, int n, const void* v1, int k1, int m, int d, int dtype,
                    const float* inv0, const float* inv1, const float* nrm0, const float* nrm1, const int* path,
                    int A, const SvxTypes& types, int W, float* costs, int* boff, int* status);
int svxl_band_costs_batch(svx_ctx*, const SvxPairDev* pairs, int n_pairs, int depth, int max_A, const SvxTypes& types,
                          int W, int dtype, int d);
bool svxl_band2_limits(const SvxTypes& types, int W, int depth, int dtype, int d, int* lim, int* tamax);
int svxl_band_costs2_batch(svx_ctx*, const SvxPairDev* pairs, int n_pairs, int depth, int max_A, const SvxTypes& types, int W,
                           int dtype, int d);
int svxl_band_tiles_shape(const SvxTypes& types);
size_t svxl_band_tiles_scratch(const SvxTypes& types);
int svxl_band_tiles_batch(svx_ctx*, const SvxPairDev* pairs, int n_pairs, const SvxTypes& types, int W, int dtype, int max_nd,
                          int* gpref, int* ticket, float* planes);
int svxl_dense_dp(svx_ctx*, const float* cost, int s0, int s1, float pen, double* csum, int* bp);
int svxl_dense_stage_batch(svx_ctx*, const SvxPairDev* pairs, int n_pairs, int max_s0);
int svxl_dense_traceback(svx_ctx*, const int* bp, int s0, int s1, int* align, int* count);
int svxl_sparse_dp(svx_ctx*, const float* costs, const int* boff_in, int A, int B, const SvxTypes& types, double pen,
                   int xs, int ys, double* csum, int* xp, int* yp, int* boff_out);
int svxl_sparse_dp_batch(svx_ctx*, const SvxPairDev* pairs, int n_pairs, int depth, const SvxTypes& types, int B);
int svxl_sparse_traceback(svx_ctx*, const double* csum, const int* xp, const int* yp, const int* boff, int a_out,
                          int B, int xs, int ys, int* align, double* scores, int* count);
int svxl_sparse_traceback_batch(svx_ctx*, const SvxPairDev* pairs, int n_pairs, int depth, int B, int max_A, int packed);
int svxl_search_path(svx_ctx*, const int* align, const int* n_align, int upsample, int size0, int size1, int* path,
                     int cap, int* path_len);
int svxl_search_path_batch(svx_ctx*, const SvxPairDev* pairs, int n_pairs, int depth, int max_rows, int max_src_rows, int chunk_lim,
                           int chunk_tamax);
int svxl_del_penalty(svx_ctx*, const float* scores, int64_t n, double frac, double* out);
int svxl_del_penalty_batch(svx_ctx*, const SvxPairDev* pairs, int n_pairs, int max_levels, double frac);
```

### speech-vecalign_amd/csrc/svx_costs.hip

```cpp
#include <stdlib.h>

#include "svx_common.h"

namespace {

typedef __attribute__((ext_vector_type(8))) __bf16 bf16x8_t;
typedef __attribute__((ext_vector_type(8))) _Float16 f16x8_t;
typedef __attribute__((ext_vector_type(4))) float f32x4_t;

constexpr int RS = 144;

template <typename E>
struct Mma;
template <>
struct Mma<ElemBF16> {
    static constexpr int KS = 64, NK = 2, KSTEP_BYTES = 64;
    using frag = uint4;
    __device__ static __forceinline__ int lane_off(int lane) { return (lane & 15) * RS + 16 * (lane >> 4); }
    __device__ static __forceinline__ frag load(const char* p) { return *reinterpret_cast<const uint4*>(p); }
    __device__ static __forceinline__ void mma(f32x4_t& acc, const frag& a, const frag& b) {
        acc = __builtin_amdgcn_mfma_f32_16x16x32_bf16(__builtin_bit_cast(bf16x8_t, a), __builtin_bit_cast(bf16x8_t, b), acc, 0, 0, 0);
    }
};
template <>
struct Mma<ElemF16> {
    static constexpr int KS = 64, NK = 2, KSTEP_BYTES = 64;
    using frag = uint4;
    __device__ static __forceinline__ int lane_off(int lane) { return (lane & 15) * RS + 16 * (lane >> 4); }
    __device__ static __forceinline__ frag load(const char* p) { return *reinterpret_cast<const uint4*>(p); }
    __device__ static __forceinline__ void mma(f32x4_t& acc, const frag& a, const frag& b) {
        acc = __builtin_amdgcn_mfma_f32_16x16x32_f16(__builtin_bit_cast(f16x8_t, a), __builtin_bit_cast(f16x8_t, b), acc, 0, 0, 0);
    }
};
template <>
struct Mma<ElemF32> {
    static constexpr int KS = 32, NK = 8, KSTEP_BYTES = 16;
    using frag = float;
    __device__ static __forceinline__ int lane_off(int lane) { return (lane & 15) * RS + 4 * (lane >> 4); }
    __device__ static __forceinline__ frag load(const char* p) { return *reinterpret_cast<const float*>(p); }
    __device__ static __forceinline__ void mma(f32x4_t& acc, const frag& a, const frag& b) {
        acc = __builtin_amdgcn_mfma_f32_16x16x4f32(a, b, acc, 0, 0, 0);
    }
};

template <typename E>
__device__ __forceinline__ void stage_slab(char* slab, const char* const* rowptr, int nrows, int k0, int d, int tid,
                                           int nthreads) {
    using S = typename E::storage;
    const int npieces = nrows * 8;
    for (int q = tid; q < npieces; q += nthreads) {
        const int r = q >> 3, p = q & 7;
        const char* ptr = rowptr[r];
        const int kel = k0 + p * E::VEC;
        uint4 v = make_uint4(0, 0, 0, 0);
        if (ptr != nullptr && kel < d) v = *reinterpret_cast<const uint4*>(ptr + (size_t)kel * sizeof(S));
        *reinterpret_cast<uint4*>(slab + r * RS + p * 16) = v;
    }
}

__device__ __forceinline__ float cost_formula(float sumx, int p, int q, float n0, float n1) {
#pragma clang fp contract(off)
    return (float)((((2.0 * (double)p) * (double)q) * (1.0 - (double)sumx)) / ((1e-6 + (double)n0) + (double)n1));
}

struct DenseArgs {
    const void* v0;
    const void* v1;
    int s0, s1, d;
    const float* inv0;
    const float* inv1;
    const float* n0;
    const float* n1;
    int mul0, mul1;
    float* costs;
    float* dots;
};

constexpr int DT = 64;
template <typename E>
__device__ void dense_block(const DenseArgs& g, int bx, int by, char* smem) {
    using S = typename E::storage;
    const int tid = threadIdx.x, lane = tid & 63, wave = tid >> 6;
    const char** rowptr = reinterpret_cast<const char**>(smem);
    char* slab = smem + 2 * DT * sizeof(char*);
    const int x0 = bx * DT, y0 = by * DT;
    if (tid < 2 * DT) {
        const int side = tid >= DT, loc = tid - side * DT;
        const int gi = (side ? y0 : x0) + loc;
        const int nn = side ? g.s1 : g.s0;
        const char* base = reinterpret_cast<const char*>(side ? g.v1 : g.v0);
        rowptr[tid] = (gi < nn) ? base + (size_t)gi * g.d * sizeof(S) : nullptr;
    }
    f32x4_t acc[2][2];
#pragma unroll
    for (int i = 0; i < 2; i++)
#pragma unroll
        for (int j = 0; j < 2; j++) acc[i][j] = (f32x4_t){0.f, 0.f, 0.f, 0.f};
    const int xt = wave >> 1, yt = wave & 1;
    for (int k0 = 0; k0 < g.d; k0 += Mma<E>::KS) {
        __syncthreads();
        stage_slab<E>(slab, rowptr, 2 * DT, k0, g.d, tid, blockDim.x);
        __syncthreads();
        const char* ap = slab + xt * 32 * RS + Mma<E>::lane_off(lane);
        const char* bp = slab + (DT + yt * 32) * RS + Mma<E>::lane_off(lane);
#pragma unroll
        for (int ks = 0; ks < Mma<E>::NK; ks++) {
            const typename Mma<E>::frag a0 = Mma<E>::load(ap + ks * Mma<E>::KSTEP_BYTES);
            const typename Mma<E>::frag a1 = Mma<E>::load(ap + 16 * RS + ks * Mma<E>::KSTEP_BYTES);
            const typename Mma<E>::frag b0 = Mma<E>::load(bp + ks * Mma<E>::KSTEP_BYTES);
            const typename Mma<E>::frag b1 = Mma<E>::load(bp + 16 * RS + ks * Mma<E>::KSTEP_BYTES);
            Mma<E>::mma(acc[0][0], a0, b0);
            Mma<E>::mma(acc[0][1], a0, b1);
            Mma<E>::mma(acc[1][0], a1, b0);
            Mma<E>::mma(acc[1][1], a1, b1);
        }
    }
#pragma unroll
    for (int i = 0; i < 2; i++)
#pragma unroll
        for (int j = 0; j < 2; j++) {
            const int y = y0 + yt * 32 + j * 16 + (lane & 15);
#pragma unroll
            for (int r = 0; r < 4; r++) {
                const int x = x0 + xt * 32 + i * 16 + (lane >> 4) * 4 + r;
                if (x < g.s0 && y < g.s1) {
                    float sumx = acc[i][j][r];
                    if (g.inv0) sumx = sumx * g.inv0[x] * g.inv1[y];
                    float c = cost_formula(sumx, 1, 1, g.n0[x], g.n1[y]);
                    c = (c * (float)g.mul0) * (float)g.mul1;
                    g.costs[(size_t)x * g.s1 + y] = c;
                    if (g.dots) g.dots[(size_t)x * g.s1 + y] = sumx;
                }
            }
        }
}

template <typename E>
__global__ __launch_bounds__(256) void k_dense_costs(DenseArgs g) {
    extern __shared__ __attribute__((aligned(16))) char smem[];
    dense_block<E>(g, blockIdx.x, blockIdx.y, smem);
}

template <typename E, bool LV0>
__global__ __launch_bounds__(256) void k_dense_costs_batch(const SvxPairDev* __restrict__ pairs) {
    extern __shared__ __attribute__((aligned(16))) char smem[];
    const SvxPairDev& P = pairs[blockIdx.z];
    if ((P.L == 0) != LV0) return;
    const SvxLevel& Lv = P.lev[P.L];
    DenseArgs g;
    g.s0 = Lv.n[0];
    g.s1 = Lv.n[1];
    if ((int)blockIdx.x * DT >= g.s0 || (int)blockIdx.y * DT >= g.s1) return;
    g.d = P.d;
    g.v0 = LV0 ? P.v[0] : (const void*)Lv.P[0];
    g.v1 = LV0 ? P.v[1] : (const void*)Lv.P[1];
    g.inv0 = LV0 ? Lv.inv[0] : nullptr;
    g.inv1 = LV0 ? Lv.inv[1] : nullptr;
    g.n0 = Lv.nrm[0];
    g.n1 = Lv.nrm[1];
    g.mul0 = 1;
    g.mul1 = 1;
    g.costs = P.dcost;
    g.dots = LV0 ? nullptr : P.ddot;
    dense_block<E>(g, blockIdx.x, blockIdx.y, smem);
}

template <typename E, int NCH>
__device__ __forceinline__ float row_dot(const typename E::storage* a, const typename E::storage* b, int d, int lane) {
    float s = 0.f;
#pragma unroll
    for (int c = 0; c < NCH; c++) {
        const int col = (c * SVX_WAVE + lane) * E::VEC;
        if (col < d) {
            float x[E::VEC], y[E::VEC];
            load_piece<E>(a + col, x);
            load_piece<E>(b + col, y);
#pragma unroll
            for (int i = 0; i < E::VEC; i++) s += x[i] * y[i];
        }
    }
    return wave_sum(s);
}

struct ScoreArgs {
    const void* v1;
    const void* v2;
    const float* inv1;
    const float* inv2;
    const float* n1;
    const float* n2;
    const int* xx;
    const int* yy;
    int64_t n;
    int rows1, rows2, d;
    float* out;
};

template <typename E, int NCH>
__device__ void score_block(const ScoreArgs& g, int64_t first, int64_t stride) {
    using S = typename E::storage;
    const int lane = threadIdx.x & 63;
    for (int64_t i = first; i < g.n; i += stride) {
        int xi = g.xx[i], yi = g.yy[i];
        xi = xi < 0 ? 0 : (xi >= g.rows1 ? g.rows1 - 1 : xi);
        yi = yi < 0 ? 0 : (yi >= g.rows2 ? g.rows2 - 1 : yi);
        float dot = row_dot<E, NCH>(reinterpret_cast<const S*>(g.v1) + (size_t)xi * g.d,
                                    reinterpret_cast<const S*>(g.v2) + (size_t)yi * g.d, g.d, lane);
        if (lane == 0) {
            if (g.inv1) dot = dot * g.inv1[xi] * g.inv2[yi];
            const float den = g.n1[xi] + g.n2[yi];
            g.out[i] = (float)((2.0 * (1.0 - (double)dot)) / (double)den);
        }
    }
}

template <typename E, int NCH>
__global__ __launch_bounds__(256) void k_score_path(ScoreArgs g) {
    score_block<E, NCH>(g, (int64_t)blockIdx.x * 4 + (threadIdx.x >> 6), (int64_t)gridDim.x * 4);
}

__device__ __forceinline__ unsigned xcd_remap(unsigned id, unsigned n);

__global__ __launch_bounds__(256) void k_knob_sort(const SvxPairDev* __restrict__ pairs) {
    extern __shared__ __attribute__((aligned(16))) char smem[];
    __shared__ int part[256];
    const SvxPairDev& P = pairs[blockIdx.y];
    const int level = blockIdx.x;
    if (level > P.L) return;
    if (P.L >= 1 && level == P.L) return;
    const SvxLevel& Lv = P.lev[level];
    const int n = Lv.n[0], kn = Lv.kn, tid = threadIdx.x;
    int* cnt = reinterpret_cast<int*>(smem);
    for (int i = tid; i < n; i += 256) cnt[i] = 0;
    __syncthreads();
    for (int i = tid; i < kn; i += 256) {
        int x = Lv.kx[i];
        x = x < 0 ? 0 : (x >= n ? n - 1 : x);
        atomicAdd(&cnt[x], 1);
    }
    __syncthreads();
    const int per = (n + 255) / 256;
    const int lo = tid * per, hi = (lo + per) < n ? (lo + per) : n;
    int sum = 0;
    for (int i = lo; i < hi; i++) sum += cnt[i];
    part[tid] = sum;
    __syncthreads();
    if (tid == 0) {
        int run = 0;
        for (int i = 0; i < 256; i++) { const int v = part[i]; part[i] = run; run += v; }
    }
    __syncthreads();
    int run = part[tid];
    for (int i = lo; i < hi; i++) {
        const int v = cnt[i];
        cnt[i] = run;
        Lv.kstart[i] = run;
        run += v;
    }
    if (tid == 0) Lv.kstart[n] = kn;
    __syncthreads();
    for (int i = tid; i < kn; i += 256) {
        int x = Lv.kx[i];
        x = x < 0 ? 0 : (x >= n ? n - 1 : x);
        const int pos = atomicAdd(&cnt[x], 1);
        const int m = Lv.n[1];
        int y = Lv.ky[i];
        y = y < 0 ? 0 : (y >= m ? m - 1 : y);
        Lv.korder[pos] = i;
        Lv.kys[pos] = y;
    }
}

constexpr int KNOB_PF = 2;

template <typename E, int NCH, bool LV0>
__global__ __launch_bounds__(256) void k_knob_scores(const SvxPairDev* __restrict__ pairs, int nlev, int bpt) {
    using S = typename E::storage;
    constexpr int EPL = NCH * E::VEC;
    const unsigned wg = xcd_remap(blockIdx.x, gridDim.x);
    const int task = wg / bpt, blk = wg % bpt;
    const SvxPairDev& P = pairs[task / nlev];
    const int level = task % nlev + (LV0 ? 0 : 1);
    if (level > P.L) return;
    if (!LV0 && level == P.L) return;
    const SvxLevel& Lv = P.lev[level];
    const int lane = threadIdx.x & 63;
    const int n = Lv.n[0], d = P.d;
    const S* v1 = LV0 ? reinterpret_cast<const S*>(P.v[0]) : reinterpret_cast<const S*>(Lv.P[0]);
    const S* v2 = LV0 ? reinterpret_cast<const S*>(P.v[1]) : reinterpret_cast<const S*>(Lv.P[1]);
    const float* inv1 = LV0 ? Lv.inv[0] : nullptr;
    const float* inv2 = LV0 ? Lv.inv[1] : nullptr;
    for (int x = blk * 4 + (threadIdx.x >> 6); x < n; x += bpt * 4) {
        const int s0 = gld(Lv.kstart + x), s1 = gld(Lv.kstart + x + 1);
        if (s0 >= s1) continue;
        float xr[EPL];
#pragma unroll
        for (int c = 0; c < NCH; c++) {
            const int col = (c * SVX_WAVE + lane) * E::VEC;
            if (col < d) {
                gload_piece<E>(v1 + (size_t)x * d + col, xr + c * E::VEC);
            } else {
#pragma unroll
                for (int i = 0; i < E::VEC; i++) xr[c * E::VEC + i] = 0.f;
            }
        }
        const float nx = gld(Lv.nrm[0] + x);
        const float ix = LV0 ? gld(inv1 + x) : 1.0f;
        constexpr int PF = KNOB_PF;
        const int ns = s1 - s0;
        for (int cb = 0; cb < ns; cb += SVX_WAVE) {
            const int cn = min(SVX_WAVE, ns - cb);
            const int ys_l = lane < cn ? gld(Lv.kys + s0 + cb + lane) : 0;
            const int is_l = lane < cn ? gld(Lv.korder + s0 + cb + lane) : 0;
            const float nrm_l = lane < cn ? gld(Lv.nrm[1] + ys_l) : 0.f;
            const float inv_l = (LV0 && lane < cn) ? gld(inv2 + ys_l) : 1.f;
            float dots_l = 0.f;
            uint4 yraw[PF][NCH];
#pragma unroll
            for (int u = 0; u < PF; u++) {
                const int yu = __builtin_amdgcn_readlane(ys_l, u);
#pragma unroll
                for (int c = 0; c < NCH; c++) {
                    const int col = (c * SVX_WAVE + lane) * E::VEC;
                    yraw[u][c] = (u < cn && col < d) ? gld16(v2 + (size_t)yu * d + col) : make_uint4(0, 0, 0, 0);
                }
            }
            for (int base = 0; base < cn; base += PF) {
#pragma unroll
                for (int u = 0; u < PF; u++) {
                    const int k = base + u;
                    if (k >= cn) break;
                    float dot = 0.f;
#pragma unroll
                    for (int c = 0; c < NCH; c++) {
                        float yr[E::VEC];
                        decode_piece<E>(yraw[u][c], yr);
#pragma unroll
                        for (int e = 0; e < E::VEC; e++) dot += xr[c * E::VEC + e] * yr[e];
                    }
                    if (k + PF < cn) {
                        const int yn = __builtin_amdgcn_readlane(ys_l, k + PF);
#pragma unroll
                        for (int c = 0; c < NCH; c++) {
                            const int col = (c * SVX_WAVE + lane) * E::VEC;
                            yraw[u][c] = col < d ? gld16(v2 + (size_t)yn * d + col) : make_uint4(0, 0, 0, 0);
                        }
                    }
                    dot = wave_sum(dot);
                    dots_l = lane == k ? dot : dots_l;
                }
            }
            if (lane < cn) {
                float dot = dots_l;
                if (LV0) dot = dot * ix * inv_l;
                const float den = nx + nrm_l;
                gst(Lv.kscore + is_l, (float)((2.0 * (1.0 - (double)dot)) / (double)den));
            }
        }
    }
}

template <typename E, int NCH, bool LV0>
__global__ __launch_bounds__(256) void k_knob_scores_unsorted(const SvxPairDev* __restrict__ pairs) {
    const SvxPairDev& P = pairs[blockIdx.z];
    const int level = (int)blockIdx.y + (LV0 ? 0 : 1);
    if (level > P.L) return;
    if (!LV0 && level == P.L) return;
    const SvxLevel& Lv = P.lev[level];
    ScoreArgs g;
    g.v1 = LV0 ? P.v[0] : (const void*)Lv.P[0];
    g.v2 = LV0 ? P.v[1] : (const void*)Lv.P[1];
    g.inv1 = LV0 ? Lv.inv[0] : nullptr;
    g.inv2 = LV0 ? Lv.inv[1] : nullptr;
    g.n1 = Lv.nrm[0];
    g.n2 = Lv.nrm[1];
    g.xx = Lv.kx;
    g.yy = Lv.ky;
    g.n = Lv.kn;
    g.rows1 = Lv.n[0];
    g.rows2 = Lv.n[1];
    g.d = P.d;
    g.out = Lv.kscore;
    score_block<E, NCH>(g, (int64_t)blockIdx.x * 4 + (threadIdx.x >> 6), (int64_t)gridDim.x * 4);
}

__global__ __launch_bounds__(256) void k_knob_from_dots(const SvxPairDev* __restrict__ pairs) {
    const SvxPairDev& P = pairs[blockIdx.y];
    if (P.L < 1) return;
    const SvxLevel& Lv = P.lev[P.L];
    const int n = Lv.n[0], m = Lv.n[1];
    for (int i = blockIdx.x * 256 + threadIdx.x; i < Lv.kn; i += gridDim.x * 256) {
        int x = Lv.kx[i], y = Lv.ky[i];
        x = x < 0 ? 0 : (x >= n ? n - 1 : x);
        y = y < 0 ? 0 : (y >= m ? m - 1 : y);
        const float dot = P.ddot[(size_t)x * m + y];
        const float den = Lv.nrm[0][x] + Lv.nrm[1][y];
        Lv.kscore[i] = (float)((2.0 * (1.0 - (double)dot)) / (double)den);
    }
}

constexpr int TA = SVX_BC_TA, TAMAX = SVX_BC_TAMAX, TB = SVX_BC_TB, ROWS = SVX_BC_ROWS;
constexpr int CPT = (TAMAX * TB + 511) / 512;
constexpr int BC_THREADS = 512;
constexpr int BC_WAVES = BC_THREADS / 64;
static_assert(BC_WAVES == 8, "unit -> (wave, slot) is decoded with shifts");
constexpr int UPW_FULL = 6;
constexpr int TPP_FULL = BC_WAVES * UPW_FULL / 3;
constexpr int DUMP_UNIT = 16 * ROWS;

struct BandArgs {
    const void* v0;
    const void* v1;
    int n, m, d;
    const float* inv0;
    const float* inv1;
    const float* nrm0;
    const float* nrm1;
    const int* path;
    int A, W;
    float* costs;
    int* boff;
    int* status;
    int atb;
};

struct BandLds {
    size_t off_rowptr, off_scal, off_work, work_bytes, total;
    int rs;
};
__host__ __device__ inline BandLds band_lds(int kx, int ky, int sw, int ntypes_pass) {
    BandLds L;
    const int NR = (kx + ky) * ROWS;
    size_t o = (2 * TAMAX + 2 * (SVX_MAX_TYPES + 2)) * sizeof(int);
    L.off_rowptr = (o + 15) & ~(size_t)15;
    o = L.off_rowptr + (size_t)NR * sizeof(char*);
    L.off_scal = (o + 15) & ~(size_t)15;
    o = L.off_scal + 2 * (size_t)NR * sizeof(float);
    L.off_work = (o + 15) & ~(size_t)15;
    L.rs = sw * 128 + 16;
    const size_t slab = (size_t)NR * L.rs;
    const size_t fs = (size_t)ntypes_pass * TAMAX * TB * sizeof(float);
    const size_t epi = fs + (size_t)BC_WAVES * DUMP_UNIT * sizeof(float);
    L.work_bytes = slab > epi ? slab : epi;
    L.total = L.off_work + L.work_bytes;
    return L;
}

template <typename E, int NPT, int SW>
__device__ __forceinline__ void slab_load(uint4* pre, const char* const* rowptr, unsigned live, int k0, int d, int tid) {
    using S = typename E::storage;
    constexpr int PPR = 8 * SW;
#pragma unroll
    for (int i = 0; i < NPT; i++) {
        const int q = tid + i * BC_THREADS;
        uint4 v = make_uint4(0, 0, 0, 0);
        if ((live >> i) & 1u) {
            const int r = q / PPR, p = q % PPR;
            const int kel = k0 + p * E::VEC;
            if (kel < d) v = *reinterpret_cast<const uint4*>(rowptr[r] + (size_t)kel * sizeof(S));
        }
        pre[i] = v;
    }
}
template <int NPT, int SW>
__device__ __forceinline__ void slab_store(const uint4* pre, char* slab, unsigned live, int tid) {
    constexpr int PPR = 8 * SW, RSB = SW * 128 + 16;
#pragma unroll
    for (int i = 0; i < NPT; i++) {
        const int q = tid + i * BC_THREADS;
        if ((live >> i) & 1u) *reinterpret_cast<uint4*>(slab + (q / PPR) * RSB + (q % PPR) * 16) = pre[i];
    }
}

template <typename E, int NPT, int SW>
__device__ void band_block(const BandArgs& g, const SvxTypes& ty, int kx, int ky, int a0, int TAe, int chunk_b, char* smem) {
    using S = typename E::storage;
    using M = Mma<E>;
    constexpr int RSB = SW * 128 + 16;
    constexpr int KSB = M::KS * SW, NKB = M::NK * SW;
    constexpr int UPW = (SW == 4) ? 1 : UPW_FULL;
    constexpr int TPP = BC_WAVES * UPW / 3;
    const int tid = threadIdx.x, lane = tid & 63, wave = tid >> 6;
    const int B = 2 * g.W;
    const int b0 = chunk_b * TB;
    const int TBe = (B - b0) < TB ? (B - b0) : TB;
    const int NR = (kx + ky) * ROWS;
    const int npieces = NR * 8 * SW;
    const BandLds L = band_lds(kx, ky, SW, ty.n < TPP ? ty.n : TPP);
    int* spx = reinterpret_cast<int*>(smem);
    int* spy = spx + TAMAX;
    int* ltx = spy + TAMAX;
    int* lty = ltx + (SVX_MAX_TYPES + 2);
    const char** rowptr = reinterpret_cast<const char**>(smem + L.off_rowptr);
    float* snrm = reinterpret_cast<float*>(smem + L.off_scal);
    float* sinv = snrm + NR;
    char* slab = smem + L.off_work;

    if (tid < TAe) {
        spx[tid] = g.path[2 * (a0 + tid)];
        spy[tid] = g.path[2 * (a0 + tid) + 1];
    }
    for (int t = tid; t < ty.n; t += BC_THREADS) {
        ltx[t] = ty.x[t];
        lty[t] = ty.y[t];
    }
    __syncthreads();
    if (tid < TAe) {
        bool ok = (spx[tid] + spy[tid] == a0 + tid);
        if (tid > 0) ok = ok && spx[tid] >= spx[tid - 1] && spy[tid] >= spy[tid - 1];
        if (!ok && g.status) *g.status = SVX_ERR_PATH;
        if (chunk_b == 0) g.boff[a0 + tid] = spy[tid] - g.W;
    }
    const int xlo = spx[0], ylo = spy[0];
    const int X0 = xlo + g.W - (b0 + TBe - 1);
    const int Y0 = ylo - g.W + b0;
    const int NXn = spx[TAe - 1] - xlo + TBe, NYn = spy[TAe - 1] - ylo + TBe;
    for (int r = tid; r < NR; r += BC_THREADS) {
        const int side = r >= kx * ROWS;
        const int rr = side ? r - kx * ROWS : r;
        const int layer = rr / ROWS, loc = rr % ROWS;
        const int gi = (side ? Y0 : X0) + loc;
        const int nn = side ? g.m : g.n;
        const bool live = loc < (side ? NYn : NXn) && gi >= 0 && gi < nn;
        const char* base = reinterpret_cast<const char*>(side ? g.v1 : g.v0);
        rowptr[r] = live ? base + ((size_t)layer * nn + gi) * g.d * sizeof(S) : nullptr;
        const float* nr = side ? g.nrm1 : g.nrm0;
        const float* iv = side ? g.inv1 : g.inv0;
        snrm[r] = live ? nr[(size_t)layer * nn + gi] : 0.f;
        sinv[r] = (live && iv) ? iv[(size_t)layer * nn + gi] : 1.f;
    }
    __syncthreads();
    const int loff = (lane & 15) * RSB + (int)(sizeof(S) == 4 ? 4 : 16) * (lane >> 4);
    unsigned live = 0;
#pragma unroll
    for (int i = 0; i < NPT; i++) {
        const int q = tid + i * BC_THREADS;
        if (q < npieces && rowptr[q / (8 * SW)] != nullptr) live |= 1u << i;
    }
    const int nxt = NXn <= 16 ? 1 : (NXn <= 32 ? 2 : 3);
    const int nyt = NYn <= 16 ? 1 : (NYn <= 32 ? 2 : 3);

    const int ncells = TAe * TBe;
    int c_ai[CPT], c_bi[CPT], c_xloc[CPT], c_yloc[CPT];
    bool c_in[CPT];
#pragma unroll
    for (int cc = 0; cc < CPT; cc++) {
        const int cell = tid + cc * BC_THREADS;
        c_ai[cc] = cell / TBe;
        c_bi[cc] = cell - c_ai[cc] * TBe;
        c_xloc[cc] = 0;
        c_yloc[cc] = 0;
        c_in[cc] = false;
        if (cell < ncells) {
            const int yy = spy[c_ai[cc]] - g.W + b0 + c_bi[cc];
            const int xx = (a0 + c_ai[cc]) - yy;
            c_xloc[cc] = xx - X0;
            c_yloc[cc] = yy - Y0;
            c_in[cc] = xx >= 0 && xx < g.n && yy >= 0 && yy < g.m;
            if (c_xloc[cc] < 0 || c_xloc[cc] >= ROWS || c_yloc[cc] < 0 || c_yloc[cc] >= ROWS) { c_xloc[cc] = 0; c_yloc[cc] = 0; c_in[cc] = false; }
        }
    }

    for (int pass = 0; pass * TPP < ty.n; pass++) {
        const int ntp = (ty.n - pass * TPP) < TPP ? (ty.n - pass * TPP) : TPP;
        const int nunits = ntp * nxt;
        const bool ksplit = nunits <= 4;
        const int khalf = ksplit ? (wave >> 2) : 0;
        f32x4_t acc[UPW][3];
        int aoff[UPW], boffs[UPW];
        int uid[UPW];
#pragma unroll
        for (int s = 0; s < UPW; s++) {
#pragma unroll
            for (int j = 0; j < 3; j++) acc[s][j] = (f32x4_t){0.f, 0.f, 0.f, 0.f};
            const int u = ksplit ? (s == 0 ? (wave & 3) : nunits) : wave + BC_WAVES * s;
            uid[s] = u;
            const int t = pass * TPP + (u < nunits ? u / nxt : 0);
            const int xt = u % nxt;
            aoff[s] = ((ltx[t] - 1) * ROWS + xt * 16) * RSB + loff;
            boffs[s] = ((kx + lty[t] - 1) * ROWS) * RSB + loff;
        }
        auto mma_slab = [&]() {
#pragma unroll
            for (int s = 0; s < UPW; s++) {
                if (uid[s] < nunits) {
                    const char* ap = slab + aoff[s];
                    const char* bp = slab + boffs[s];
                    if (ksplit) {
#pragma unroll
                        for (int ks2 = 0; ks2 < NKB / 2; ks2++) {
                            const int ko = (2 * ks2 + khalf) * M::KSTEP_BYTES;
                            const typename M::frag fa = M::load(ap + ko);
#pragma unroll
                            for (int j = 0; j < 3; j++)
                                if (j < nyt) M::mma(acc[s][j], fa, M::load(bp + j * 16 * RSB + ko));
                        }
                    } else {
#pragma unroll
                        for (int ks = 0; ks < NKB; ks++) {
                            const typename M::frag fa = M::load(ap + ks * M::KSTEP_BYTES);
#pragma unroll
                            for (int j = 0; j < 3; j++)
                                if (j < nyt) M::mma(acc[s][j], fa, M::load(bp + j * 16 * RSB + ks * M::KSTEP_BYTES));
                        }
                    }
                }
            }
        };
        if constexpr (SW == 1) {
            uint4 preA[NPT], preB[NPT];
            slab_load<E, NPT, SW>(preA, rowptr, live, 0, g.d, tid);
            __syncthreads();
            slab_store<NPT, SW>(preA, slab, live, tid);
            if (KSB < g.d) slab_load<E, NPT, SW>(preA, rowptr, live, KSB, g.d, tid);
            __syncthreads();
            for (int k0 = 0; k0 < g.d; k0 += 2 * KSB) {
                if (k0 + 2 * KSB < g.d) slab_load<E, NPT, SW>(preB, rowptr, live, k0 + 2 * KSB, g.d, tid);
                __builtin_amdgcn_sched_barrier(0);
                mma_slab();
                __syncthreads();
                if (k0 + KSB < g.d) {
                    slab_store<NPT, SW>(preA, slab, live, tid);
                    __syncthreads();
                    if (k0 + 3 * KSB < g.d) slab_load<E, NPT, SW>(preA, rowptr, live, k0 + 3 * KSB, g.d, tid);
                    __builtin_amdgcn_sched_barrier(0);
                    mma_slab();
                    __syncthreads();
                    if (k0 + 2 * KSB < g.d) slab_store<NPT, SW>(preB, slab, live, tid);
                    __syncthreads();
                }
            }
        } else {
            uint4 pre[NPT];
            slab_load<E, NPT, SW>(pre, rowptr, live, 0, g.d, tid);
            __syncthreads();
            slab_store<NPT, SW>(pre, slab, live, tid);
            __syncthreads();
            for (int k0 = 0; k0 < g.d; k0 += KSB) {
                const bool more = k0 + KSB < g.d;
                if (more) slab_load<E, NPT, SW>(pre, rowptr, live, k0 + KSB, g.d, tid);
                __builtin_amdgcn_sched_barrier(0);
                mma_slab();
                __syncthreads();
                if (more) slab_store<NPT, SW>(pre, slab, live, tid);
                __syncthreads();
            }
        }
        float* Fs = reinterpret_cast<float*>(slab);
        float* dump = Fs + (size_t)ntp * TAMAX * TB;
        const int du = (int)((L.work_bytes - (size_t)ntp * TAMAX * TB * sizeof(float)) / (DUMP_UNIT * sizeof(float)));
        const int SR = du / BC_WAVES >= UPW ? UPW : (du / BC_WAVES < 1 ? 1 : du / BC_WAVES);
        const int nslots = (nunits + BC_WAVES - 1) / BC_WAVES;
        for (int s0 = 0; s0 < nslots; s0 += SR) {
#pragma unroll
            for (int s = 0; s < UPW; s++) {
                if (s >= s0 && s < s0 + SR && uid[s] < nunits) {
                    float* dw = dump + ((s - s0) * BC_WAVES + wave) * DUMP_UNIT;
#pragma unroll
                    for (int yt = 0; yt < 3; yt++)
#pragma unroll
                        for (int r = 0; r < 4; r++) dw[((lane >> 4) * 4 + r) * ROWS + yt * 16 + (lane & 15)] = acc[s][yt][r];
                }
            }
            __syncthreads();
#pragma unroll
            for (int cc = 0; cc < CPT; cc++) {
                if (tid + cc * BC_THREADS >= ncells) continue;
                const int xq = c_xloc[cc] >> 4;
                const int ulo = s0 * BC_WAVES, uhi = (s0 + SR) * BC_WAVES < nunits ? (s0 + SR) * BC_WAVES : nunits;
                for (int tl = (ulo - xq + nxt - 1) / nxt; nxt * tl + xq < uhi; tl++) {
                    const int u = nxt * tl + xq;
                    const int t = pass * TPP + tl;
                    const int p = ltx[t], q = lty[t];
                    float c = __builtin_inff();
                    if (c_in[cc]) {
                        const int rx = (p - 1) * ROWS + c_xloc[cc], ry = (kx + q - 1) * ROWS + c_yloc[cc];
                        float dsum = dump[(u - ulo) * DUMP_UNIT + (c_xloc[cc] & 15) * ROWS + c_yloc[cc]];
                        if (ksplit) dsum += dump[(u - ulo + 4) * DUMP_UNIT + (c_xloc[cc] & 15) * ROWS + c_yloc[cc]];
                        const float sumx = dsum * sinv[rx] * sinv[ry];
                        c = cost_formula(sumx, p, q, snrm[rx], snrm[ry]);
                    }
                    Fs[((size_t)c_ai[cc] * ntp + tl) * TB + c_bi[cc]] = c;
                }
            }
            __syncthreads();
        }
        const int nout = TAe * ntp * TBe;
        for (int idx = tid; idx < nout; idx += BC_THREADS) {
            const int ai = idx / (ntp * TBe);
            const int rem = idx - ai * (ntp * TBe);
            const int tl = rem / TBe, bi = rem - tl * TBe;
            const int t = pass * TPP + tl;
            const size_t o = g.atb ? ((size_t)(a0 + ai) * ty.n + t) * B + (b0 + bi) : ((size_t)t * g.A + (a0 + ai)) * B + (b0 + bi);
            g.costs[o] = Fs[((size_t)ai * ntp + tl) * TB + bi];
        }
    }
}

template <typename E, int NPT, int SW>
__global__ __launch_bounds__(BC_THREADS) void k_band_costs(BandArgs g, SvxTypes ty, int kx, int ky, int nchunk_b) {
    extern __shared__ __attribute__((aligned(16))) char smem[];
    const int a0 = (blockIdx.x / nchunk_b) * TA;
    band_block<E, NPT, SW>(g, ty, kx, ky, a0, (g.A - a0) < TA ? (g.A - a0) : TA, blockIdx.x % nchunk_b, smem);
}

__device__ __forceinline__ unsigned xcd_remap(unsigned id, unsigned n) {
    const unsigned q = n / 8, r = n % 8, xcd = id % 8, k = id / 8;
    return (xcd < r ? xcd * (q + 1) : r * (q + 1) + (xcd - r) * q) + k;
}

template <typename E, bool LV0, int NPT, int SW>
__global__ __launch_bounds__(BC_THREADS) void k_band_costs_batch(const SvxPairDev* __restrict__ pairs, int depth, SvxTypes ty,
                                                                 int kx, int ky, int W, int nchunk_b, int per_pair) {
    extern __shared__ __attribute__((aligned(16))) char smem[];
    const unsigned wg = xcd_remap(blockIdx.x, gridDim.x);
    const SvxPairDev& P = pairs[wg / per_pair];
    const int item = wg % per_pair;
    if (depth > P.L || (depth == P.L && P.L > 0)) return;
    const SvxLevel& Lv = P.lev[depth];
    BandArgs g;
    g.A = *Lv.path_len;
    const int chunk_a = item / nchunk_b;
    if (g.A <= 0 || chunk_a >= *Lv.nchunks) return;
    const int a0 = Lv.cstart[chunk_a], TAe = Lv.cstart[chunk_a + 1] - a0;
    g.n = Lv.n[0];
    g.m = Lv.n[1];
    g.d = P.d;
    g.v0 = LV0 ? P.v[0] : (const void*)Lv.P[0];
    g.v1 = LV0 ? P.v[1] : (const void*)Lv.P[1];
    g.inv0 = LV0 ? Lv.inv[0] : nullptr;
    g.inv1 = LV0 ? Lv.inv[1] : nullptr;
    g.nrm0 = Lv.nrm[0];
    g.nrm1 = Lv.nrm[1];
    g.path = Lv.path;
    g.W = W;
    g.costs = Lv.costs;
    g.boff = Lv.boff;
    g.status = P.status;
    g.atb = 1;
    band_block<E, NPT, SW>(g, ty, kx, ky, a0, TAe, item % nchunk_b, smem);
}

inline int nch_f32(int d) {
    int c = (d + 255) / 256;
    return c <= 1 ? 1 : c <= 2 ? 2 : c <= 4 ? 4 : 8;
}
inline int nch_16(int d) {
    int c = (d + 511) / 512;
    return c <= 1 ? 1 : c <= 2 ? 2 : 4;
}

constexpr size_t DENSE_SMEM = 2 * DT * sizeof(char*) + 2 * DT * RS;

}

int svxl_dense_costs(svx_ctx* ctx, const float* v0, int s0, const float* v1, int s1, int d, const float* n0,
                     const float* n1, int mul0, int mul1, float* costs) {
    if (s0 <= 0 || s1 <= 0) return SVX_OK;
    DenseArgs g{v0, v1, s0, s1, d, nullptr, nullptr, n0, n1, mul0, mul1, costs, nullptr};
    hipLaunchKernelGGL(k_dense_costs<ElemF32>, dim3((s0 + DT - 1) / DT, (s1 + DT - 1) / DT), dim3(256), DENSE_SMEM, ctx->stream, g);
    SVX_LAUNCH_CHECK(ctx, "k_dense_costs");
    return SVX_OK;
}

int svxl_dense_costs_batch(svx_ctx* ctx, const SvxPairDev* pairs, int n_pairs, int max_s0, int max_s1, int dtype, int d) {
    (void)d;
    if (n_pairs <= 0 || max_s0 <= 0 || max_s1 <= 0) return SVX_OK;
    dim3 grid((max_s0 + DT - 1) / DT, (max_s1 + DT - 1) / DT, n_pairs);
    hipLaunchKernelGGL((k_dense_costs_batch<ElemF32, false>), grid, dim3(256), DENSE_SMEM, ctx->stream, pairs);
    if (dtype == SVX_F32)
        hipLaunchKernelGGL((k_dense_costs_batch<ElemF32, true>), grid, dim3(256), DENSE_SMEM, ctx->stream, pairs);
    else if (dtype == SVX_F16)
        hipLaunchKernelGGL((k_dense_costs_batch<ElemF16, true>), grid, dim3(256), DENSE_SMEM, ctx->stream, pairs);
    else
        hipLaunchKernelGGL((k_dense_costs_batch<ElemBF16, true>), grid, dim3(256), DENSE_SMEM, ctx->stream, pairs);
    SVX_LAUNCH_CHECK(ctx, "k_dense_costs_batch");
    return SVX_OK;
}

int svxl_score_path(svx_ctx* ctx, const int* xx, const int* yy, int64_t n, const float* n1, const float* n2,
                    const float* v1, int rows1, const float* v2, int rows2, int d, float* out) {
    if (n <= 0) return SVX_OK;
    ScoreArgs g{v1, v2, nullptr, nullptr, n1, n2, xx, yy, n, rows1, rows2, d, out};
    int64_t nb = (n + 3) / 4;
    if (nb > 16384) nb = 16384;
#define M(N) hipLaunchKernelGGL((k_score_path<ElemF32, N>), dim3((unsigned)nb), dim3(256), 0, ctx->stream, g)
    switch (nch_f32(d)) {
        case 1: M(1); break;
        case 2: M(2); break;
        case 4: M(4); break;
        default: M(8); break;
    }
#undef M
    SVX_LAUNCH_CHECK(ctx, "k_score_path");
    return SVX_OK;
}

int svxl_knob_from_dots(svx_ctx* ctx, const SvxPairDev* pairs, int n_pairs, int max_kn) {
    if (n_pairs <= 0 || max_kn <= 0) return SVX_OK;
    int nb = (max_kn + 255) / 256;
    if (nb > 16) nb = 16;
    hipLaunchKernelGGL(k_knob_from_dots, dim3(nb, n_pairs), dim3(256), 0, ctx->stream, pairs);
    SVX_LAUNCH_CHECK(ctx, "k_knob_from_dots");
    return SVX_OK;
}

int svxl_knob_scores(svx_ctx* ctx, const SvxPairDev* pairs, int n_pairs, int max_L, int max_kn, int max_n0, int dtype, int d,
                     int part) {
    if (n_pairs <= 0 || max_kn <= 0) return SVX_OK;
    hipStream_t st = ctx->stream;
    const bool unsorted = (size_t)(max_n0 + 1) * sizeof(int) > 150 * 1024;
    if (unsorted) {
        if (part == 0) return SVX_OK;
        const int nbu = (max_kn + 3) / 4 < 2048 ? (max_kn + 3) / 4 : 2048;
#define U32(N, LV0, GY) hipLaunchKernelGGL((k_knob_scores_unsorted<ElemF32, N, LV0>), dim3(nbu, GY, n_pairs), dim3(256), 0, st, pairs)
#define U16(E, N) hipLaunchKernelGGL((k_knob_scores_unsorted<E, N, true>), dim3(nbu, 1, n_pairs), dim3(256), 0, st, pairs)
        if (part == 1) {
            if (max_L >= 1) {
                switch (nch_f32(d)) {
                    case 1: U32(1, false, max_L); break;
                    case 2: U32(2, false, max_L); break;
                    case 4: U32(4, false, max_L); break;
                    default: U32(8, false, max_L); break;
                }
            }
        } else if (dtype == SVX_F32) {
            switch (nch_f32(d)) {
                case 1: U32(1, true, 1); break;
                case 2: U32(2, true, 1); break;
                case 4: U32(4, true, 1); break;
                default: U32(8, true, 1); break;
            }
        } else if (dtype == SVX_F16) {
            switch (nch_16(d)) {
                case 1: U16(ElemF16, 1); break;
                case 2: U16(ElemF16, 2); break;
                default: U16(ElemF16, 4); break;
            }
        } else {
            switch (nch_16(d)) {
                case 1: U16(ElemBF16, 1); break;
                case 2: U16(ElemBF16, 2); break;
                default: U16(ElemBF16, 4); break;
            }
        }
#undef U32
#undef U16
        SVX_LAUNCH_CHECK(ctx, "k_knob_scores_unsorted");
        return SVX_OK;
    }
    if (part == 0) {
        const size_t smem = (size_t)(max_n0 + 1) * sizeof(int);
        if (smem > 64 * 1024)
            SVX_HIP(ctx, hipFuncSetAttribute((const void*)k_knob_sort, hipFuncAttributeMaxDynamicSharedMemorySize, (int)smem));
        hipLaunchKernelGGL(k_knob_sort, dim3(max_L + 1, n_pairs), dim3(256), smem, st, pairs);
        SVX_LAUNCH_CHECK(ctx, "k_knob_sort");
        return SVX_OK;
    }
    int nb = (max_n0 + 3) / 4;
    if (nb > 1024) nb = 1024;
#define M32(N, LV0, GY) hipLaunchKernelGGL((k_knob_scores<ElemF32, N, LV0>), dim3((unsigned)nb * (GY) * n_pairs), dim3(256), 0, st, pairs, GY, nb)
#define M16(E, N) hipLaunchKernelGGL((k_knob_scores<E, N, true>), dim3((unsigned)nb * n_pairs), dim3(256), 0, st, pairs, 1, nb)
    if (part == 1 && max_L >= 1) {
        switch (nch_f32(d)) {
            case 1: M32(1, false, max_L); break;
            case 2: M32(2, false, max_L); break;
            case 4: M32(4, false, max_L); break;
            default: M32(8, false, max_L); break;
        }
    }
    if (part != 2) {
    } else if (dtype == SVX_F32) {
        switch (nch_f32(d)) {
            case 1: M32(1, true, 1); break;
            case 2: M32(2, true, 1); break;
            case 4: M32(4, true, 1); break;
            default: M32(8, true, 1); break;
        }
    } else if (dtype == SVX_F16) {
        switch (nch_16(d)) {
            case 1: M16(ElemF16, 1); break;
            case 2: M16(ElemF16, 2); break;
            default: M16(ElemF16, 4); break;
        }
    } else {
        switch (nch_16(d)) {
            case 1: M16(ElemBF16, 1); break;
            case 2: M16(ElemBF16, 2); break;
            default: M16(ElemBF16, 4); break;
        }
    }
#undef M32
#undef M16
    SVX_LAUNCH_CHECK(ctx, "k_knob_scores");
    return SVX_OK;
}

static int types_layers(const SvxTypes& ty, int* kx, int* ky) {
    int mx = 0, my = 0;
    for (int t = 0; t < ty.n; t++) {
        if (ty.x[t] > mx) mx = ty.x[t];
        if (ty.y[t] > my) my = ty.y[t];
    }
    *kx = mx;
    *ky = my;
    return 0;
}

struct BandPlan {
    int sw, npt;
    size_t smem;
};

static int band_plan(svx_ctx* ctx, int kx, int ky, int ntypes, BandPlan* bp) {
    const int NR = (kx + ky) * ROWS;
    const char* sw_env = getenv("SVX_BAND_SW");
    const int sw_max = sw_env ? atoi(sw_env) : 4;
    for (int sw = 4; sw >= 1; sw >>= 1) {
        if (sw > sw_max) continue;
        const int tpp = sw == 4 ? BC_WAVES / 3 : TPP_FULL;
        const int ntp = ntypes < tpp ? ntypes : tpp;
        if (sw == 4 && ntypes > tpp) continue;
        const BandLds L = band_lds(kx, ky, sw, ntp);
        const int npt = (NR * 8 * sw + BC_THREADS - 1) / BC_THREADS;
        if (sw == 4 && (NR > 2 * ROWS || L.total > 64 * 1024)) continue;
        if (sw == 2 && (L.total > 128 * 1024 || npt > 12)) continue;
        if (L.total > 160 * 1024 || npt > 14)
            return svx_fail(ctx, SVX_ERR_ARG, "band costs: %d+%d overlap layers need %zu bytes of LDS / %d staging pieces (limits 160 KiB / 14)",
                            kx, ky, L.total, npt);
        bp->sw = sw;
        bp->npt = npt < 1 ? 1 : npt;
        bp->smem = L.total;
        return SVX_OK;
    }
    return svx_fail(ctx, SVX_ERR_ARG, "band costs: no launch configuration");
}

#define BAND_DISPATCH(CALL)                      \
    do {                                         \
        if (bp.sw == 4) {                        \
            CALL(6, 4);                          \
        } else if (bp.sw == 2) {                 \
            if (bp.npt <= 3) CALL(3, 2);         \
            else if (bp.npt <= 6) CALL(6, 2);    \
            else CALL(12, 2);                    \
        } else {                                 \
            if (bp.npt <= 2) CALL(2, 1);         \
            else if (bp.npt <= 6) CALL(6, 1);    \
            else if (bp.npt <= 8) CALL(8, 1);    \
            else CALL(14, 1);                    \
        }                                        \
    } while (0)

int svxl_band_costs(svx_ctx* ctx, const void* v0, int k0, int n, const void* v1, int k1, int m, int d, int dtype,
                    const float* inv0, const float* inv1, const float* nrm0, const float* nrm1, const int* path, int A,
                    const SvxTypes& types, int W, float* costs, int* boff, int* status) {
    if (A <= 0) return SVX_OK;
    int kx, ky;
    types_layers(types, &kx, &ky);
    if (kx > k0 || ky > k1) return svx_fail(ctx, SVX_ERR_OVERLAPS, "overlaps");
    if (types.n == 0) kx = ky = 0;
    BandPlan bp;
    int rc = band_plan(ctx, kx, ky, types.n, &bp);
    if (rc) return rc;
    const size_t smem = bp.smem;
    const int B = 2 * W;
    const int nca = (A + TA - 1) / TA, ncb = (B + TB - 1) / TB;
    BandArgs g{v0, v1, n, m, d, inv0, inv1, nrm0, nrm1, path, A, W, costs, boff, status, 0};
    dim3 grid((unsigned)(nca * ncb));
#define CALL_E(E, NPT, SW)                                                                                          \
    do {                                                                                                            \
        if (smem > 64 * 1024)                                                                                       \
            SVX_HIP(ctx, hipFuncSetAttribute((const void*)k_band_costs<E, NPT, SW>, hipFuncAttributeMaxDynamicSharedMemorySize, (int)smem)); \
        hipLaunchKernelGGL((k_band_costs<E, NPT, SW>), grid, dim3(BC_THREADS), smem, ctx->stream, g, types, kx, ky, ncb); \
    } while (0)
#define CALL_F32(NPT, SW) CALL_E(ElemF32, NPT, SW)
#define CALL_F16(NPT, SW) CALL_E(ElemF16, NPT, SW)
#define CALL_BF16(NPT, SW) CALL_E(ElemBF16, NPT, SW)
    if (dtype == SVX_F32) BAND_DISPATCH(CALL_F32);
    else if (dtype == SVX_F16) BAND_DISPATCH(CALL_F16);
    else BAND_DISPATCH(CALL_BF16);
#undef CALL_F32
#undef CALL_F16
#undef CALL_BF16
#undef CALL_E
    SVX_LAUNCH_CHECK(ctx, "k_band_costs");
    return SVX_OK;
}

int svxl_band_costs_batch(svx_ctx* ctx, const SvxPairDev* pairs, int n_pairs, int depth, int max_A, const SvxTypes& types,
                          int W, int dtype, int d) {
    (void)d;
    if (n_pairs <= 0 || max_A <= 0) return SVX_OK;
    int kx, ky;
    types_layers(types, &kx, &ky);
    if (types.n == 0) kx = ky = 0;
    BandPlan bp;
    int rc = band_plan(ctx, kx, ky, types.n, &bp);
    if (rc) return rc;
    const size_t smem = bp.smem;
    const int B = 2 * W;
    const int nca = (max_A + TA - 1) / TA, ncb = (B + TB - 1) / TB;
    const int per_pair = nca * ncb;
    dim3 grid((unsigned)per_pair * (unsigned)n_pairs);
#define CALL_E(E, LV0, NPT, SW)                                                                                     \
    do {                                                                                                            \
        if (smem > 64 * 1024)                                                                                       \
            SVX_HIP(ctx, hipFuncSetAttribute((const void*)k_band_costs_batch<E, LV0, NPT, SW>, hipFuncAttributeMaxDynamicSharedMemorySize, (int)smem)); \
        hipLaunchKernelGGL((k_band_costs_batch<E, LV0, NPT, SW>), grid, dim3(BC_THREADS), smem, ctx->stream, pairs, depth, types, kx, ky, W, ncb, per_pair); \
    } while (0)
#define CALL_DEEP(NPT, SW) CALL_E(ElemF32, false, NPT, SW)
#define CALL_F32(NPT, SW) CALL_E(ElemF32, true, NPT, SW)
#define CALL_F16(NPT, SW) CALL_E(ElemF16, true, NPT, SW)
#define CALL_BF16(NPT, SW) CALL_E(ElemBF16, true, NPT, SW)
    if (depth > 0) BAND_DISPATCH(CALL_DEEP);
    else if (dtype == SVX_F32) BAND_DISPATCH(CALL_F32);
    else if (dtype == SVX_F16) BAND_DISPATCH(CALL_F16);
    else BAND_DISPATCH(CALL_BF16);
#undef CALL_DEEP
#undef CALL_F32
#undef CALL_F16
#undef CALL_BF16
#undef CALL_E
    SVX_LAUNCH_CHECK(ctx, "k_band_costs_batch");
    return SVX_OK;
}
```

### speech-vecalign_amd/svx/_lib.py

```python
import ctypes
import os
import threading

_HERE = os.path.dirname(os.path.abspath(__file__))
LIB_PATH = os.environ.get("SVX_LIB") or os.path.join(_HERE, "libsvx.so")

SVX_F32, SVX_F16, SVX_BF16 = 0, 1, 2
SVX_MAX_TYPES = 128
SVX_MAX_LEVELS = 16
SVX_MARGIN_RATIO, SVX_MARGIN_DISTANCE, SVX_MARGIN_ABSOLUTE = 0, 1, 2
SVX_SEARCH_COARSE_TO_FINE, SVX_SEARCH_STRAIGHT = 0, 1

SVX_OK, SVX_ERR_ARG, SVX_ERR_OVERLAPS, SVX_ERR_HIP, SVX_ERR_TRACEBACK = 0, 1, 2, 3, 4
SVX_ERR_NOMEM, SVX_ERR_EXTEND, SVX_ERR_PATH, SVX_ERR_BP = 5, 6, 7, 8

DEVICE_ERRORS = {
    SVX_ERR_TRACEBACK: "traceback bug",
    SVX_ERR_BP: "got unknown value",
    SVX_ERR_EXTEND: "asked to extend alignments but already bigger than requested",
    SVX_ERR_PATH: "search path is not a unit-step lattice path",
}

c_int, c_i64, c_f32, c_f64, c_vp = ctypes.c_int, ctypes.c_int64, ctypes.c_float, ctypes.c_double, ctypes.c_void_p


class AlignParams(ctypes.Structure):
    _fields_ = [
        ("dtype", ctypes.c_int32),
        ("d", ctypes.c_int32),
        ("n_types", ctypes.c_int32),
        ("types", ctypes.c_int32 * (2 * SVX_MAX_TYPES)),
        ("width_over2", ctypes.c_int32),
        ("max_size_full_dp", ctypes.c_int32),
        ("costs_sample_size", ctypes.c_int32),
        ("num_samps_for_norm", ctypes.c_int32),
        ("del_percentile_frac", ctypes.c_double),
        ("search_mode", ctypes.c_int32),
        ("reserved0", ctypes.c_int32),
    ]


class LevelView(ctypes.Structure):
    _fields_ = [
        ("size0", ctypes.c_int32), ("size1", ctypes.c_int32), ("k0", ctypes.c_int32), ("k1", ctypes.c_int32),
        ("n_types", ctypes.c_int32), ("band", ctypes.c_int32), ("path_len", ctypes.c_int32), ("n_align", ctypes.c_int32),
        ("n0", c_vp), ("n1", c_vp), ("del_penalty", c_vp), ("searchpath", c_vp), ("a_b_costs", c_vp), ("b_offset", c_vp),
        ("a_b_csum", c_vp), ("a_b_bp", c_vp), ("a_b_xp", c_vp), ("a_b_yp", c_vp), ("new_b_offset", c_vp),
        ("alignments", c_vp), ("alignment_scores", c_vp),
        ("costs_1to1", c_vp), ("x_y_tb_diag", c_vp), ("v0_l0", c_vp), ("v1_l0", c_vp),
        ("knob_scores", c_vp), ("n_knob", ctypes.c_int32), ("reserved", ctypes.c_int32),
    ]


class Pair(ctypes.Structure):
    _fields_ = [
        ("vecs0", c_vp), ("vecs1", c_vp),
        ("n", ctypes.c_int32), ("m", ctypes.c_int32), ("k0", ctypes.c_int32), ("k1", ctypes.c_int32),
        ("norm_idx", c_vp), ("knob_idx", c_vp),
        ("norms0", c_vp), ("norms1", c_vp),
        ("align", c_vp), ("scores", c_vp), ("info", c_vp), ("del_pen", c_vp),
    ]


class Frames(ctypes.Structure):
    _fields_ = [("src", c_vp), ("tgt", c_vp)]


class ConcatParams(ctypes.Structure):
    _fields_ = [
        ("max_score", ctypes.c_double),
        ("max_num_align", ctypes.c_int32), ("sample_rate", ctypes.c_int32),
        ("max_sil", ctypes.c_double), ("max_dur", ctypes.c_double),
        ("both_sides", ctypes.c_int32), ("pad", ctypes.c_int32),
        ("min_frames", ctypes.c_int64),
    ]


SVX_CONCAT_MAX = 8

_SIGS = {
    "svx_create": (c_int, [c_int, ctypes.POINTER(c_vp)]),
    "svx_destroy": (c_int, [c_vp]),
    "svx_set_stream": (c_int, [c_vp, c_vp]),
    "svx_synchronize": (c_int, [c_vp]),
    "svx_last_error": (ctypes.c_char_p, [c_vp]),
    "svx_version": (ctypes.c_char_p, []),
    "svx_scratch_bytes": (c_i64, [c_vp]),
    "svx_dense_costs": (c_int, [c_vp, c_vp, c_int, c_int, c_vp, c_int, c_int, c_int, c_vp, c_vp, c_int, c_int, c_vp]),
    "svx_dense_dp": (c_int, [c_vp, c_vp, c_int, c_int, c_f32, c_vp, c_vp]),
    "svx_score_path": (c_int, [c_vp, c_vp, c_vp, c_i64, c_vp, c_vp, c_vp, c_int, c_vp, c_int, c_int, c_vp]),
    "svx_sparse_costs": (c_int, [c_vp, c_vp, c_int, c_int, c_vp, c_int, c_int, c_int, c_vp, c_vp, c_vp, c_int,
                                 ctypes.POINTER(ctypes.c_int32), c_int, c_int, c_vp, c_vp]),
    "svx_sparse_dp": (c_int, [c_vp, c_vp, c_vp, c_int, c_int, ctypes.POINTER(ctypes.c_int32), c_int, c_f64, c_int, c_int,
                              c_vp, c_vp, c_vp, c_vp]),
    "svx_make_norm1": (c_int, [c_vp, c_vp, c_i64, c_int]),
    "svx_downsample": (c_int, [c_vp, c_vp, c_int, c_int, c_int, c_vp]),
    "svx_compute_norms": (c_int, [c_vp, c_vp, c_int, c_int, c_vp, c_int, c_int, c_int, c_vp, c_int, c_vp]),
    "svx_del_penalty": (c_int, [c_vp, c_vp, c_i64, c_f64, c_vp]),
    "svx_dense_traceback": (c_int, [c_vp, c_vp, c_int, c_int, c_vp, c_vp]),
    "svx_sparse_traceback": (c_int, [c_vp, c_vp, c_vp, c_vp, c_vp, c_int, c_int, c_int, c_int, c_vp, c_vp, c_vp]),
    "svx_search_path": (c_int, [c_vp, c_vp, c_vp, c_int, c_int, c_int, c_vp, c_vp]),
    "svx_gather_rows": (c_int, [c_vp, c_vp, c_i64, c_int, c_int, c_vp, c_i64, c_vp]),
    "svx_unit_rows": (c_int, [c_vp, c_vp, c_int, c_i64, c_int, c_vp, c_int]),
    "svx_knn_mean_sim": (c_int, [c_vp, c_vp, c_int, c_i64, c_vp, c_int, c_i64, c_int, c_int, c_vp]),
    "svx_knn_topk_merge": (c_int, [c_vp, c_vp, c_int, c_i64, c_vp, c_int, c_i64, c_int, c_int, c_vp, c_int, c_vp]),
    "svx_knn_search": (c_int, [c_vp, c_vp, c_int, c_i64, c_vp, c_int, c_i64, c_int, c_int, c_i64, c_vp, c_vp, c_int]),
    "svx_knn_search_groups": (c_int, [c_vp, c_vp, c_int, c_vp, c_int, c_int, c_int, c_vp, c_vp, c_int, c_vp, c_vp]),
    "svx_margin_scores": (c_int, [c_vp, c_vp, c_vp, c_int, c_i64, c_int, c_vp, c_vp, c_int, c_vp]),
    "svx_knn_list_means": (c_int, [c_vp, c_vp, c_i64, c_int, c_vp]),
    "svx_margin_candidates": (c_int, [c_vp, c_vp, c_vp, c_i64, c_int, c_vp, c_vp, c_i64, c_i64, c_int, c_vp, c_vp, c_vp]),
    "svx_mine_greedy": (c_i64, [c_vp, c_i64, c_vp, c_vp, c_i64, c_i64, c_vp]),
    "svx_mt19937_choice": (c_int, [c_vp, ctypes.POINTER(ctypes.c_int32), c_i64, c_i64, c_vp]),
    "svx_norm_index_count": (c_i64, [c_int, c_int, c_int, c_int, c_int, c_int, c_int, c_int]),
    "svx_knob_index_count": (c_i64, [c_int, c_int, c_int, c_int]),
    "svx_draw_indices": (c_int, [c_vp, ctypes.POINTER(ctypes.c_int32), c_int, c_int, c_int, c_int, c_int, c_int, c_int, c_int, c_int,
                                 c_vp, c_vp]),
    "svx_candidate_table": (c_int, [ctypes.c_char_p, ctypes.c_char_p, ctypes.c_char_p, c_int, c_vp, c_int,
                                    ctypes.POINTER(ctypes.c_int32), ctypes.POINTER(c_i64), ctypes.c_char_p, c_int]),
    "svx_format_alignments": (c_i64, [c_vp, c_vp, c_i64, c_vp, c_i64]),
    "svx_num_levels": (c_int, [c_int, c_int, c_int]),
    "svx_knob_count": (c_i64, [c_int, c_int, c_int]),
    "svx_align_batch": (c_int, [c_vp, ctypes.POINTER(AlignParams), ctypes.POINTER(Pair), c_int]),
    "svx_alignment_rows": (c_int, [c_vp, c_int, c_int, ctypes.POINTER(Pair), c_int, c_f64, c_i64, c_vp, c_vp, c_vp, c_vp, c_int, c_vp, c_vp]),
    "svx_concat_rows": (c_int, [c_vp, c_int, c_int, ctypes.POINTER(Pair), ctypes.POINTER(Frames), c_int, ctypes.POINTER(ConcatParams), c_i64,
                                c_vp, c_vp, c_vp, c_vp, c_int, c_vp, c_vp]),
    "svx_debug_level": (c_int, [c_vp, c_int, c_int, ctypes.POINTER(LevelView)]),
    "svx_copy_to_host": (c_int, [c_vp, c_vp, c_vp, c_i64]),
    "svx_set_profiling": (c_int, [c_vp, c_int]),
    "svx_set_pipeline": (c_int, [c_vp, c_int]),
    "svx_flush": (c_int, [c_vp]),
    "svx_stage_ms": (c_f64, [c_vp, ctypes.c_char_p]),
    "svx_stage_launches": (c_int, [c_vp, ctypes.c_char_p]),
}

EXPORTS = tuple(_SIGS)

_lib = None
_lock = threading.Lock()


def load():
    global _lib
    with _lock:
        if _lib is None:
            if not os.path.exists(LIB_PATH):
                raise ImportError(
                    "libsvx.so not found at %s: build it with `make -C speech-vecalign_amd/csrc` "
                    "(there is no CPU fallback)" % LIB_PATH)
            L = ctypes.CDLL(LIB_PATH)
            for name, (res, args) in _SIGS.items():
                fn = getattr(L, name)
                fn.restype = res
                fn.argtypes = args
            _lib = L
    return _lib


class SvxError(Exception):
    def __init__(self, code, msg):
        super().__init__(msg)
        self.code = code


class Context:

    def __init__(self, device=0):
        import torch
        if not torch.cuda.is_available():
            raise RuntimeError("svx needs a HIP device (torch.cuda.is_available() is False); there is no CPU fallback")
        self.lib = load()
        self.device = int(device)
        h = c_vp()
        rc = self.lib.svx_create(self.device, ctypes.byref(h))
        if rc != 0:
            raise SvxError(rc, self.lib.svx_last_error(None).decode())
        self.h = h
        self.torch = torch
        self.tdev = torch.device("cuda", self.device)
        self.pipeline = False
        self._held = []
        if os.environ.get("SVX_PIPELINE") == "1":
            self.set_pipeline(True)

    def use_current_stream(self):
        self.lib.svx_set_stream(self.h, c_vp(self.torch.cuda.current_stream(self.tdev).cuda_stream))

    def check(self, rc):
        if rc != 0:
            msg = self.lib.svx_last_error(self.h).decode()
            if rc == SVX_ERR_OVERLAPS:
                raise Exception(msg)
            raise SvxError(rc, msg)

    def sync(self):
        self.check(self.lib.svx_synchronize(self.h))
        del self._held[:]

    def set_pipeline(self, on):
        if self._held:
            self.flush()
        self.check(self.lib.svx_set_pipeline(self.h, 1 if on else 0))
        self.pipeline = bool(on)

    def flush(self):
        self.check(self.lib.svx_flush(self.h))
        del self._held[:]

    def hold(self, batch):
        if self.pipeline and not any(b is batch for b in self._held):
            if len(self._held) >= 4:
                self.flush()
            self._held.append(batch)

    def __del__(self):
        try:
            if getattr(self, "h", None):
                self.lib.svx_destroy(self.h)
                self.h = None
        except Exception:
            pass


_ctxs = {}


def context(device=None):
    if device is None:
        import torch
        if not torch.cuda.is_available():
            raise RuntimeError("svx needs a HIP device (torch.cuda.is_available() is False); there is no CPU fallback")
        device = torch.cuda.current_device()
    device = int(device)
    if device not in _ctxs:
        _ctxs[device] = Context(device)
    c = _ctxs[device]
    c.use_current_stream()
    return c
```

Measured before the change: 9667 doc-pairs/s.

## Launch second-half knob sort early on side stream, add one-pass knob sort kernel

```diff
diff --git a/include/svx.h b/include/svx.h
--- a/include/svx.h
+++ b/include/svx.h
@@ -155,6 +155,7 @@
 int64_t svx_knob_count(int n_l, int m_l, int costs_sample_size);
 
 int svx_align_batch(svx_ctx *ctx, const svx_align_params *params, const svx_pair *pairs, int n_pairs);
+int svx_check_batch(const svx_align_params *params, const svx_pair *pairs, int n_pairs);
 
 int svx_alignment_rows(svx_ctx *ctx, int dtype, int d, const svx_pair *pairs, int n_pairs, double max_score, int64_t cap,
                        void *x_rows, void *y_rows, void *x_unit, void *y_unit, int unit_dtype, int32_t *src, int64_t *count);
@@ -194,6 +195,9 @@
     const float *v0_l0, *v1_l0;
     const float *knob_scores;
     int32_t n_knob, reserved;
+    const int32_t *knob_start;
+    const int32_t *knob_order;
+    const int32_t *knob_ys;
 } svx_level_view;
 int svx_debug_level(svx_ctx *ctx, int pair, int level, svx_level_view *out);
 int svx_copy_to_host(svx_ctx *ctx, void *dst_host, const void *src_device, int64_t bytes);
diff --git a/speech-vecalign_amd/csrc/svx_api.hip b/speech-vecalign_amd/csrc/svx_api.hip
--- a/speech-vecalign_amd/csrc/svx_api.hip
+++ b/speech-vecalign_amd/csrc/svx_api.hip
@@ -63,6 +63,9 @@
     bool chain_done_valid = false;
     hipEvent_t front_done = nullptr, chain_done = nullptr, upload_done = nullptr;
     bool upload_valid = false;
+    hipEvent_t gathers_start = nullptr;
+    hipEvent_t early_done = nullptr;
+    bool early = false;
 };
 
 struct svx_ctx_ext : svx_ctx {
@@ -180,6 +183,8 @@
         if (H.front_done) (void)hipEventDestroy(H.front_done);
         if (H.chain_done) (void)hipEventDestroy(H.chain_done);
         if (H.upload_done) (void)hipEventDestroy(H.upload_done);
+        if (H.gathers_start) (void)hipEventDestroy(H.gathers_start);
+        if (H.early_done) (void)hipEventDestroy(H.early_done);
     }
     delete c;
     return SVX_OK;
@@ -527,11 +532,74 @@
     }
     out->knob_scores = Lv.kscore;
     out->n_knob = Lv.kn;
+    if (!(level == P.L && P.L >= 1) && !svx_knob_unsorted((second ? cx->half[1] : cx->half[0]).max_n0)) {
+        out->knob_start = Lv.kstart;
+        out->knob_order = Lv.korder;
+        out->knob_ys = Lv.kys;
+    }
     if (level >= 1) {
         out->v0_l0 = Lv.P[0];
         out->v1_l0 = Lv.P[1];
     }
     return SVX_OK;
+}
+
+static int batch_params(svx_ctx* ctx, const svx_align_params* prm, BatchParams* out) {
+    BatchParams& bp = *out;
+    int rc = check_dim(ctx, prm->d);
+    if (rc) return rc;
+    bp.d = prm->d;
+    bp.dtype = prm->dtype;
+    NEED(ctx, bp.dtype == SVX_F32 || bp.dtype == SVX_F16 || bp.dtype == SVX_BF16, "svx_align_batch: unknown dtype %d", bp.dtype);
+    NEED(ctx, prm->max_size_full_dp >= 1, "svx_align_batch: max_size_full_dp must be >= 1");
+    NEED(ctx, prm->costs_sample_size >= 1, "svx_align_batch: costs_sample_size must be >= 1");
+    NEED(ctx, prm->num_samps_for_norm >= 0, "svx_align_batch: num_samps_for_norm must be >= 0");
+    if ((rc = make_types(ctx, prm->types, prm->n_types, &bp.tfinal))) return rc;
+    const int32_t one_one[2] = {1, 1};
+    make_types(ctx, one_one, 1, &bp.t11);
+    bp.W = prm->width_over2 < 3 ? 3 : prm->width_over2;
+    bp.B = 2 * bp.W;
+    bp.nsamp = prm->num_samps_for_norm;
+    bp.frac = prm->del_percentile_frac;
+    bp.n_types = bp.tfinal.n;
+    int mx = 0, my = 0;
+    for (int t = 0; t < bp.tfinal.n; t++) { if (bp.tfinal.x[t] > mx) mx = bp.tfinal.x[t]; if (bp.tfinal.y[t] > my) my = bp.tfinal.y[t]; }
+    bp.packable = mx <= 15 && my <= 15;
+    NEED(ctx, prm->search_mode == SVX_SEARCH_COARSE_TO_FINE || prm->search_mode == SVX_SEARCH_STRAIGHT, "svx_align_batch: unknown search_mode %d", prm->search_mode);
+    bp.straight = prm->search_mode == SVX_SEARCH_STRAIGHT;
+    bp.tiles = bp.straight && bp.B > 64;
+    if (bp.tiles) NEED(ctx, bp.tfinal.n >= 1 && svxl_band_tiles_shape(bp.tfinal) >= 0, "wide straight band: no tile shape takes these %d alignment types", bp.tfinal.n);
+    return SVX_OK;
+}
+
+static int validate_pairs(svx_ctx* ctx, const BatchParams& bp, const svx_align_params* prm, const svx_pair* pairs, int n_pairs) {
+    int mx = 0, my = 0;
+    for (int t = 0; t < bp.tfinal.n; t++) { if (bp.tfinal.x[t] > mx) mx = bp.tfinal.x[t]; if (bp.tfinal.y[t] > my) my = bp.tfinal.y[t]; }
+    for (int p = 0; p < n_pairs; p++) {
+        const svx_pair& in = pairs[p];
+        NEED(ctx, in.vecs0 && in.vecs1 && in.align && in.scores && in.info && in.knob_idx, "pair %d: null pointer", p);
+        NEED(ctx, in.n >= 1 && in.m >= 1 && in.k0 >= 1 && in.k1 >= 1, "pair %d: empty document or no overlap layers", p);
+        if (mx > in.k0) return svx_fail(ctx, SVX_ERR_OVERLAPS, "%d x overlaps requrested (via alignment_types), but vecs0 only has %d", mx, in.k0);
+        if (my > in.k1) return svx_fail(ctx, SVX_ERR_OVERLAPS, "%d y overlaps requrested (via alignment_types), but vecs1 only has %d", my, in.k1);
+        const int L = bp.straight ? 0 : svx_num_levels(in.n, in.m, prm->max_size_full_dp);
+        NEED(ctx, L < SVX_MAX_LEVELS, "pair %d: %d pyramid levels (max %d)", p, L + 1, SVX_MAX_LEVELS);
+        if (bp.nsamp > 0 && (L >= 1 || !in.norms0 || !in.norms1)) NEED(ctx, in.norm_idx != nullptr, "pair %d: norm_idx is NULL", p);
+        if (bp.tiles) {
+            const long long TI = in.n / 32 + 1, TJ = in.m / 32 + 1, nd = TI + TJ - 1;
+            long long tcap = nd * ((bp.B + 64) / 32 + 2);
+            if (tcap > TI * TJ) tcap = TI * TJ;
+            NEED(ctx, tcap < (1ll << 30), "pair %d: too many tiles", p);
+        }
+    }
+    return SVX_OK;
+}
+
+extern "C" int svx_check_batch(const svx_align_params* prm, const svx_pair* pairs, int n_pairs) {
+    NEED(nullptr, prm && (pairs || n_pairs <= 0), "svx_check_batch: null argument");
+    BatchParams bp;
+    int rc = batch_params(nullptr, prm, &bp);
+    if (rc) return rc;
+    return validate_pairs(nullptr, bp, prm, pairs, n_pairs);
 }
 
 static int plan_half(svx_ctx* ctx, HalfState& H, const BatchParams& bp, const svx_align_params* prm, const svx_pair* pairs, int n_pairs) {
@@ -540,12 +608,11 @@
     const SvxTypes& tfinal = bp.tfinal;
     const int B = bp.B;
     const bool straight = bp.straight, tiles = bp.tiles, packable = bp.packable;
-    int mx = 0, my = 0;
-    for (int t = 0; t < tfinal.n; t++) { if (tfinal.x[t] > mx) mx = tfinal.x[t]; if (tfinal.y[t] > my) my = tfinal.y[t]; }
     std::vector<SvxPairDev>& host = H.host;
     host.assign(n_pairs, SvxPairDev());
     H.n_pairs = n_pairs;
     H.bp = bp;
+    H.early = false;
     H.maxL = H.max_ksum = H.max_kn = H.max_ds0 = H.max_ds1 = H.max_n0 = H.max_tnd = 0;
     H.any_L0 = false;
     H.o_tickets = 0;
@@ -559,13 +626,8 @@
         const svx_pair& in = pairs[p];
         SvxPairDev& P = host[p];
         memset(&P, 0, sizeof(P));
-        NEED(ctx, in.vecs0 && in.vecs1 && in.align && in.scores && in.info && in.knob_idx, "pair %d: null pointer", p);
-        NEED(ctx, in.n >= 1 && in.m >= 1 && in.k0 >= 1 && in.k1 >= 1, "pair %d: empty document or no overlap layers", p);
-        if (mx > in.k0) return svx_fail(ctx, SVX_ERR_OVERLAPS, "%d x overlaps requrested (via alignment_types), but vecs0 only has %d", mx, in.k0);
-        if (my > in.k1) return svx_fail(ctx, SVX_ERR_OVERLAPS, "%d y overlaps requrested (via alignment_types), but vecs1 only has %d", my, in.k1);
         const int L = straight ? 0 : svx_num_levels(in.n, in.m, prm->max_size_full_dp);
         P.straight = straight ? 1 : 0;
-        NEED(ctx, L < SVX_MAX_LEVELS, "pair %d: %d pyramid levels (max %d)", p, L + 1, SVX_MAX_LEVELS);
         P.v[0] = in.vecs0; P.v[1] = in.vecs1;
         P.K[0] = in.k0; P.K[1] = in.k1;
         P.L = L; P.d = d;
@@ -593,7 +655,6 @@
                 Lv.S[s] = skip ? 0 : S_from[s];
                 Lv.sidx[s] = nullptr;
                 if (Lv.S[s] > 0) {
-                    NEED(ctx, nidx != nullptr, "pair %d: norm_idx is NULL", p);
                     Lv.sidx[s] = nidx;
                     nidx += (size_t)K[s] * Lv.S[s];
                 }
@@ -680,7 +741,6 @@
             P.t_nd = (int)(TI + TJ - 1);
             long long tcap = (long long)P.t_nd * ((B + 64) / 32 + 2);
             if (tcap > TI * TJ) tcap = TI * TJ;
-            NEED(ctx, tcap < (1ll << 30), "pair %d: too many tiles", p);
             P.t_cap = (int)tcap;
             OFF(P.t_lo, (size_t)P.t_nd * sizeof(int));
             OFF(P.t_cnt, (size_t)P.t_nd * sizeof(int));
@@ -809,7 +869,8 @@
         SVX_HIP(ctx, hipEventRecord(cx->side_join, inline_sort ? main_stream : cx->side));
         return SVX_OK;
     };
-    if (parts == 1) ops.push_back({0.0, -1, sort_op});
+    const bool sort_here = !H.early;
+    if (parts == 1 && sort_here) ops.push_back({0.0, -1, sort_op});
     for (int l = 0; l <= H.maxL; l++) {
         for (int q = 0; q < parts; q++) {
             const int lo = (int)((long long)np * q / parts), hi = (int)((long long)np * (q + 1) / parts);
@@ -846,17 +907,18 @@
                 return SVX_OK;
             }});
         }
-        if (parts > 1 && l == 0) ops.push_back({0.0, -1, sort_op});
+        if (parts > 1 && l == 0 && sort_here) ops.push_back({0.0, -1, sort_op});
     }
     if (!bp.straight) {
         ops.push_back({H.dense_cells * 2.7e-5, S_DENSE_COSTS, [=]() -> int {
-            int rc = svxl_dense_costs_batch(ctx, h->dpairs, np, h->max_ds0, h->max_ds1, dtype, d);
+            int rc = svxl_dense_costs_batch(ctx, h->dpairs, np, h->max_ds0, h->max_ds1, dtype, d, h->maxL >= 1, h->any_L0);
             if (rc) return rc;
             return svxl_knob_from_dots(ctx, h->dpairs, np, h->max_kn);
         }});
     }
     if (H.maxL >= 1) {
         ops.push_back({H.b_knobN / 16.5e6, S_KNOB_SCORES, [=]() -> int {
+            SVX_HIP(ctx, hipEventRecord(h->gathers_start, ctx->stream));
             SVX_HIP(ctx, hipStreamWaitEvent(ctx->stream, cx->side_join, 0));
             return svxl_knob_scores(ctx, h->dpairs, np, h->maxL, h->max_kn, h->max_n0, dtype, d, 1);
         }});
@@ -938,7 +1000,51 @@
         if (!cx->half[h].front_done) SVX_HIP(ctx, hipEventCreateWithFlags(&cx->half[h].front_done, hipEventDisableTiming));
         if (!cx->half[h].chain_done) SVX_HIP(ctx, hipEventCreateWithFlags(&cx->half[h].chain_done, hipEventDisableTiming));
         if (!cx->half[h].upload_done) SVX_HIP(ctx, hipEventCreateWithFlags(&cx->half[h].upload_done, hipEventDisableTiming));
-    }
+        if (!cx->half[h].gathers_start) SVX_HIP(ctx, hipEventCreateWithFlags(&cx->half[h].gathers_start, hipEventDisableTiming));
+        if (!cx->half[h].early_done) SVX_HIP(ctx, hipEventCreateWithFlags(&cx->half[h].early_done, hipEventDisableTiming));
+    }
+    return SVX_OK;
+}
+
+static int upload_and_init(svx_ctx* ctx, HalfState& H) {
+    StageScope sc(ctx, S_SETUP);
+    hipStream_t st = ctx->stream;
+    if (H.upload_valid) SVX_HIP(ctx, hipEventSynchronize(H.upload_done));
+    memcpy(H.pinned, H.host.data(), (size_t)H.n_pairs * sizeof(SvxPairDev));
+    SVX_HIP(ctx, hipMemcpyAsync(H.dpairs, H.pinned, (size_t)H.n_pairs * sizeof(SvxPairDev), hipMemcpyHostToDevice, st));
+    SVX_HIP(ctx, hipEventRecord(H.upload_done, st));
+    H.upload_valid = true;
+    hipLaunchKernelGGL(k_init_batch, dim3(H.n_pairs), dim3(64), 0, st, H.dpairs);
+    SVX_LAUNCH_CHECK(ctx, "k_init_batch");
+    if (H.bp.nsamp == 0) {
+        for (int p = 0; p < H.n_pairs; p++)
+            for (int l = 0; l <= H.host[p].L; l++)
+                for (int s = 0; s < 2; s++)
+                    SVX_HIP(ctx, hipMemsetAsync(H.host[p].lev[l].rbar[s], 0, (size_t)H.bp.d * sizeof(float), st));
+    }
+    return SVX_OK;
+}
+
+static int launch_early(svx_ctx* ctx, HalfState& H, HalfState& first) {
+    svx_ctx_ext* cx = X(ctx);
+    const char* env = getenv("SVX_SORT_EARLY");
+    if ((env && atoi(env) == 0) || getenv("SVX_SORT_INLINE") != nullptr || first.maxL < 1) return SVX_OK;
+    hipStream_t keep = ctx->stream;
+    if (H.chain_done_valid) SVX_HIP(ctx, hipStreamWaitEvent(cx->side, H.chain_done, 0));
+    SVX_HIP(ctx, hipStreamWaitEvent(cx->side, first.gathers_start, 0));
+    ctx->stream = cx->side;
+    int rc = upload_and_init(ctx, H);
+    hipError_t e = hipSuccess;
+    if (!rc) {
+        e = hipEventRecord(H.early_done, cx->side);
+        StageScope sc(ctx, S_KNOB_SORT);
+        rc = svxl_knob_scores(ctx, H.dpairs, H.n_pairs, H.maxL, H.max_kn, H.max_n0, H.bp.dtype, H.bp.d, 0);
+    }
+    ctx->stream = keep;
+    if (rc) return rc;
+    SVX_HIP(ctx, e);
+    SVX_HIP(ctx, hipEventRecord(cx->side_join, cx->side));
+    H.early = true;
     return SVX_OK;
 }
 
@@ -949,22 +1055,9 @@
     std::vector<Seg> segs;
     if (front) {
         if (front->chain_done_valid) SVX_HIP(ctx, hipStreamWaitEvent(A, front->chain_done, 0));
-        {
-            StageScope sc(ctx, S_SETUP);
-            if (front->upload_valid) SVX_HIP(ctx, hipEventSynchronize(front->upload_done));
-            memcpy(front->pinned, front->host.data(), (size_t)front->n_pairs * sizeof(SvxPairDev));
-            SVX_HIP(ctx, hipMemcpyAsync(front->dpairs, front->pinned, (size_t)front->n_pairs * sizeof(SvxPairDev), hipMemcpyHostToDevice, A));
-            SVX_HIP(ctx, hipEventRecord(front->upload_done, A));
-            front->upload_valid = true;
-            hipLaunchKernelGGL(k_init_batch, dim3(front->n_pairs), dim3(64), 0, A, front->dpairs);
-            SVX_LAUNCH_CHECK(ctx, "k_init_batch");
-            if (front->bp.nsamp == 0) {
-                for (int p = 0; p < front->n_pairs; p++)
-                    for (int l = 0; l <= front->host[p].L; l++)
-                        for (int s = 0; s < 2; s++)
-                            SVX_HIP(ctx, hipMemsetAsync(front->host[p].lev[l].rbar[s], 0, (size_t)front->bp.d * sizeof(float), A));
-            }
-        }
+        int rc0;
+        if (front->early) SVX_HIP(ctx, hipStreamWaitEvent(A, front->early_done, 0));
+        else if ((rc0 = upload_and_init(ctx, *front))) return rc0;
         static const int split_env = [] { const char* e = getenv("SVX_PIPE_SPLIT"); const int v = e ? atoi(e) : 2; return v >= 1 && v <= 8 ? v : 2; }();
         front_ops(ctx, *front, fops, beside ? split_env : 1);
     }
@@ -1034,31 +1127,11 @@
     if (n_pairs <= 0) return SVX_OK;
     const auto t_enter = std::chrono::steady_clock::now();
     svx_ctx_ext* cx = X(ctx);
+    BatchParams bp;
+    int rc = batch_params(ctx, prm, &bp);
+    if (rc) return rc;
+    if ((rc = validate_pairs(ctx, bp, prm, pairs, n_pairs))) return rc;
     SVX_HIP(ctx, hipSetDevice(ctx->device));
-    int rc = check_dim(ctx, prm->d);
-    if (rc) return rc;
-    BatchParams bp;
-    bp.d = prm->d;
-    bp.dtype = prm->dtype;
-    NEED(ctx, bp.dtype == SVX_F32 || bp.dtype == SVX_F16 || bp.dtype == SVX_BF16, "svx_align_batch: unknown dtype %d", bp.dtype);
-    NEED(ctx, prm->max_size_full_dp >= 1, "svx_align_batch: max_size_full_dp must be >= 1");
-    NEED(ctx, prm->costs_sample_size >= 1, "svx_align_batch: costs_sample_size must be >= 1");
-    NEED(ctx, prm->num_samps_for_norm >= 0, "svx_align_batch: num_samps_for_norm must be >= 0");
-    if ((rc = make_types(ctx, prm->types, prm->n_types, &bp.tfinal))) return rc;
-    const int32_t one_one[2] = {1, 1};
-    make_types(ctx, one_one, 1, &bp.t11);
-    bp.W = prm->width_over2 < 3 ? 3 : prm->width_over2;
-    bp.B = 2 * bp.W;
-    bp.nsamp = prm->num_samps_for_norm;
-    bp.frac = prm->del_percentile_frac;
-    bp.n_types = bp.tfinal.n;
-    int mx = 0, my = 0;
-    for (int t = 0; t < bp.tfinal.n; t++) { if (bp.tfinal.x[t] > mx) mx = bp.tfinal.x[t]; if (bp.tfinal.y[t] > my) my = bp.tfinal.y[t]; }
-    bp.packable = mx <= 15 && my <= 15;
-    NEED(ctx, prm->search_mode == SVX_SEARCH_COARSE_TO_FINE || prm->search_mode == SVX_SEARCH_STRAIGHT, "svx_align_batch: unknown search_mode %d", prm->search_mode);
-    bp.straight = prm->search_mode == SVX_SEARCH_STRAIGHT;
-    bp.tiles = bp.straight && bp.B > 64;
-    if (bp.tiles) NEED(ctx, bp.tfinal.n >= 1 && svxl_band_tiles_shape(bp.tfinal) >= 0, "wide straight band: no tile shape takes these %d alignment types", bp.tfinal.n);
     if ((rc = ensure_streams(ctx))) return rc;
     for (int i = 0; i < S_COUNT; i++) { cx->ms[i] = 0.0; cx->launches[i] = 0; }
     for (auto& r : cx->recs) { (void)hipEventDestroy(r.a); (void)hipEventDestroy(r.b); }
@@ -1088,6 +1161,7 @@
             if ((rc = plan_half(ctx, H1, bp, prm, pairs + n0, n_pairs - n0))) return rc;
             plan_ms += std::chrono::duration<double, std::milli>(std::chrono::steady_clock::now() - t0).count();
             cx->last_split = n0;
+            if ((rc = launch_early(ctx, H1, H0))) return rc;
             if ((rc = run_interleaved(ctx, &H1, &H0, true))) return rc;
         }
     }
diff --git a/speech-vecalign_amd/csrc/svx_common.h b/speech-vecalign_amd/csrc/svx_common.h
--- a/speech-vecalign_amd/csrc/svx_common.h
+++ b/speech-vecalign_amd/csrc/svx_common.h
@@ -257,11 +257,13 @@
                        int max_ksum, int part);
 int svxl_score_path(svx_ctx*, const int* xx, const int* yy, int64_t n, const float* n1, const float* n2,
                     const float* v1, int rows1, const float* v2, int rows2, int d, float* out);
+static inline bool svx_knob_unsorted(int max_n0) { return (size_t)(max_n0 + 1) * sizeof(int) > 150 * 1024; }
 int svxl_knob_scores(svx_ctx*, const SvxPairDev* pairs, int n_pairs, int max_levels, int max_kn, int max_n0, int dtype, int d,
                      int part);
 int svxl_dense_costs(svx_ctx*, const float* v0, int s0, const float* v1, int s1, int d, const float* n0,
                      const float* n1, int mul0, int mul1, float* costs);
-int svxl_dense_costs_batch(svx_ctx*, const SvxPairDev* pairs, int n_pairs, int max_s0, int max_s1, int dtype, int d);
+int svxl_dense_costs_batch(svx_ctx*, const SvxPairDev* pairs, int n_pairs, int max_s0, int max_s1, int dtype, int d,
+                           bool any_deep, bool any_L0);
 int svxl_knob_from_dots(svx_ctx*, const SvxPairDev* pairs, int n_pairs, int max_kn);
 int svxl_band_costs(svx_ctx*, const void* v0, int k0, int n, const void* v1, int k1, int m, int d, int dtype,
                     const float* inv0, const float* inv1, const float* nrm0, const float* nrm1, const int* path,
diff --git a/speech-vecalign_amd/csrc/svx_costs.hip b/speech-vecalign_amd/csrc/svx_costs.hip
--- a/speech-vecalign_amd/csrc/svx_costs.hip
+++ b/speech-vecalign_amd/csrc/svx_costs.hip
@@ -269,6 +269,108 @@
         Lv.korder[pos] = i;
         Lv.kys[pos] = y;
     }
+}
+
+constexpr int KS1_THREADS = 512, KS1_VEC = 10;
+constexpr int KS1_CAP = KS1_THREADS * KS1_VEC * 4 - 3;
+constexpr int KS1_MAX_ROWS = 65536;
+static_assert(KS1_CAP < 32768, "the rank of a sample is packed in 15 bits");
+__global__ __launch_bounds__(KS1_THREADS) void k_knob_sort1(const SvxPairDev* __restrict__ pairs) {
+    extern __shared__ __attribute__((aligned(16))) char smem[];
+    __shared__ int part[256];
+    const SvxPairDev& P = pairs[blockIdx.y];
+    const int level = blockIdx.x;
+    if (level > P.L) return;
+    if (P.L >= 1 && level == P.L) return;
+    const SvxLevel& Lv = P.lev[level];
+    const int n = Lv.n[0], m = Lv.n[1], kn = Lv.kn, tid = threadIdx.x;
+    const int ax = (int)((reinterpret_cast<uintptr_t>(Lv.kx) >> 2) & 3), ay = (int)((reinterpret_cast<uintptr_t>(Lv.ky) >> 2) & 3);
+    const int* kxa = Lv.kx - ax;
+    const int nvec = (kn + ax + 3) >> 2;
+    uint4 xv[KS1_VEC];
+#pragma unroll
+    for (int g = 0; g < KS1_VEC; g++) {
+        const int q = g * KS1_THREADS + tid;
+        xv[g] = q < nvec ? gld16(kxa + 4 * q) : make_uint4(0, 0, 0, 0);
+    }
+    int* cnt = reinterpret_cast<int*>(smem);
+    for (int i = tid; i < n; i += KS1_THREADS) cnt[i] = 0;
+    __syncthreads();
+    unsigned pk[KS1_VEC * 4];
+    const int idle_row = tid < n ? tid : 0;
+#pragma unroll
+    for (int s = 0; s < KS1_VEC * 4; s++) {
+        const int i = 4 * ((s >> 2) * KS1_THREADS + tid) + (s & 3) - ax;
+        const bool live = (unsigned)i < (unsigned)kn;
+        const uint4 v = xv[s >> 2];
+        int x = (int)((s & 3) == 0 ? v.x : (s & 3) == 1 ? v.y : (s & 3) == 2 ? v.z : v.w);
+        x = x < 0 ? 0 : (x >= n ? n - 1 : x);
+        const unsigned rank = (unsigned)atomicAdd(&cnt[live ? x : idle_row], live ? 1 : 0);
+        pk[s] = live ? ((unsigned)x | (rank << 16)) : 0xffffffffu;
+    }
+    int yy[KS1_VEC * 4];
+    if (ay == ax) {
+        const int* kya = Lv.ky - ax;
+#pragma unroll
+        for (int g = 0; g < KS1_VEC; g++) {
+            const int q = g * KS1_THREADS + tid;
+            const uint4 v = q < nvec ? gld16(kya + 4 * q) : make_uint4(0, 0, 0, 0);
+            yy[4 * g] = (int)v.x; yy[4 * g + 1] = (int)v.y; yy[4 * g + 2] = (int)v.z; yy[4 * g + 3] = (int)v.w;
+        }
+    } else {
+#pragma unroll
+        for (int s = 0; s < KS1_VEC * 4; s++) {
+            const int i = 4 * ((s >> 2) * KS1_THREADS + tid) + (s & 3) - ax;
+            yy[s] = (unsigned)i < (unsigned)kn ? gld(Lv.ky + i) : 0;
+        }
+    }
+    __syncthreads();
+    const int per = (n + 255) / 256;
+    const int lo = tid * per, hi = (lo + per) < n ? (lo + per) : n;
+    if (tid < 256) {
+        int sum = 0;
+        for (int i = lo; i < hi; i++) sum += cnt[i];
+        part[tid] = sum;
+    }
+    __syncthreads();
+    if (tid == 0) {
+        int run = 0;
+        for (int i = 0; i < 256; i++) { const int v = part[i]; part[i] = run; run += v; }
+    }
+    __syncthreads();
+    if (tid < 256) {
+        int run = part[tid];
+        for (int i = lo; i < hi; i++) {
+            const int v = cnt[i];
+            cnt[i] = run;
+            Lv.kstart[i] = run;
+            run += v;
+        }
+    }
+    if (tid == 0) Lv.kstart[n] = kn;
+    __syncthreads();
+#pragma unroll
+    for (int s = 0; s < KS1_VEC * 4; s++) {
+        const bool live = pk[s] != 0xffffffffu;
+        const int first = cnt[live ? (pk[s] & 0xffffu) : 0u];
+        pk[s] = live ? (unsigned)first + (pk[s] >> 16) : 0xffffffffu;
+    }
+    asm volatile("" ::: "memory");
+#pragma unroll
+    for (int s = 0; s < KS1_VEC * 4; s++) {
+        if (pk[s] == 0xffffffffu) continue;
+        const int i = 4 * ((s >> 2) * KS1_THREADS + tid) + (s & 3) - ax;
+        int y = yy[s];
+        y = y < 0 ? 0 : (y >= m ? m - 1 : y);
+        Lv.korder[pk[s]] = i;
+        Lv.kys[pk[s]] = y;
+    }
+}
+
+static bool knob_sort_one_pass(int max_kn, int max_n0) {
+    const char* env = getenv("SVX_KNOB_SORT_V");
+    if (env && atoi(env) <= 1) return false;
+    return max_kn <= KS1_CAP && max_n0 < KS1_MAX_ROWS;
 }
 
 constexpr int KNOB_PF = 2;
@@ -763,12 +865,14 @@
     return SVX_OK;
 }
 
-int svxl_dense_costs_batch(svx_ctx* ctx, const SvxPairDev* pairs, int n_pairs, int max_s0, int max_s1, int dtype, int d) {
+int svxl_dense_costs_batch(svx_ctx* ctx, const SvxPairDev* pairs, int n_pairs, int max_s0, int max_s1, int dtype, int d,
+                           bool any_deep, bool any_L0) {
     (void)d;
     if (n_pairs <= 0 || max_s0 <= 0 || max_s1 <= 0) return SVX_OK;
     dim3 grid((max_s0 + DT - 1) / DT, (max_s1 + DT - 1) / DT, n_pairs);
-    hipLaunchKernelGGL((k_dense_costs_batch<ElemF32, false>), grid, dim3(256), DENSE_SMEM, ctx->stream, pairs);
-    if (dtype == SVX_F32)
+    if (any_deep) hipLaunchKernelGGL((k_dense_costs_batch<ElemF32, false>), grid, dim3(256), DENSE_SMEM, ctx->stream, pairs);
+    if (!any_L0) {
+    } else if (dtype == SVX_F32)
         hipLaunchKernelGGL((k_dense_costs_batch<ElemF32, true>), grid, dim3(256), DENSE_SMEM, ctx->stream, pairs);
     else if (dtype == SVX_F16)
         hipLaunchKernelGGL((k_dense_costs_batch<ElemF16, true>), grid, dim3(256), DENSE_SMEM, ctx->stream, pairs);
@@ -809,7 +913,7 @@
                      int part) {
     if (n_pairs <= 0 || max_kn <= 0) return SVX_OK;
     hipStream_t st = ctx->stream;
-    const bool unsorted = (size_t)(max_n0 + 1) * sizeof(int) > 150 * 1024;
+    const bool unsorted = svx_knob_unsorted(max_n0);
     if (unsorted) {
         if (part == 0) return SVX_OK;
         const int nbu = (max_kn + 3) / 4 < 2048 ? (max_kn + 3) / 4 : 2048;
@@ -851,9 +955,12 @@
     }
     if (part == 0) {
         const size_t smem = (size_t)(max_n0 + 1) * sizeof(int);
+        const bool one_pass = knob_sort_one_pass(max_kn, max_n0);
         if (smem > 64 * 1024)
-            SVX_HIP(ctx, hipFuncSetAttribute((const void*)k_knob_sort, hipFuncAttributeMaxDynamicSharedMemorySize, (int)smem));
-        hipLaunchKernelGGL(k_knob_sort, dim3(max_L + 1, n_pairs), dim3(256), smem, st, pairs);
+            SVX_HIP(ctx, hipFuncSetAttribute(one_pass ? (const void*)k_knob_sort1 : (const void*)k_knob_sort,
+                                             hipFuncAttributeMaxDynamicSharedMemorySize, (int)smem));
+        if (one_pass) hipLaunchKernelGGL(k_knob_sort1, dim3(max_L + 1, n_pairs), dim3(KS1_THREADS), smem, st, pairs);
+        else hipLaunchKernelGGL(k_knob_sort, dim3(max_L + 1, n_pairs), dim3(256), smem, st, pairs);
         SVX_LAUNCH_CHECK(ctx, "k_knob_sort");
         return SVX_OK;
     }
@@ -861,7 +968,7 @@
     if (nb > 1024) nb = 1024;
 #define M32(N, LV0, GY) hipLaunchKernelGGL((k_knob_scores<ElemF32, N, LV0>), dim3((unsigned)nb * (GY) * n_pairs), dim3(256), 0, st, pairs, GY, nb)
 #define M16(E, N) hipLaunchKernelGGL((k_knob_scores<E, N, true>), dim3((unsigned)nb * n_pairs), dim3(256), 0, st, pairs, 1, nb)
-    if (part == 1 && max_L >= 1) {
+    if (part == 1 && max_L >= 2) {
         switch (nch_f32(d)) {
             case 1: M32(1, false, max_L); break;
             case 2: M32(2, false, max_L); break;
diff --git a/speech-vecalign_amd/svx/_lib.py b/speech-vecalign_amd/svx/_lib.py
--- a/speech-vecalign_amd/svx/_lib.py
+++ b/speech-vecalign_amd/svx/_lib.py
@@ -49,6 +49,7 @@
         ("alignments", c_vp), ("alignment_scores", c_vp),
         ("costs_1to1", c_vp), ("x_y_tb_diag", c_vp), ("v0_l0", c_vp), ("v1_l0", c_vp),
         ("knob_scores", c_vp), ("n_knob", ctypes.c_int32), ("reserved", ctypes.c_int32),
+        ("knob_start", c_vp), ("knob_order", c_vp), ("knob_ys", c_vp),
     ]
 
 
@@ -121,6 +122,7 @@
     "svx_num_levels": (c_int, [c_int, c_int, c_int]),
     "svx_knob_count": (c_i64, [c_int, c_int, c_int]),
     "svx_align_batch": (c_int, [c_vp, ctypes.POINTER(AlignParams), ctypes.POINTER(Pair), c_int]),
+    "svx_check_batch": (c_int, [ctypes.POINTER(AlignParams), ctypes.POINTER(Pair), c_int]),
     "svx_alignment_rows": (c_int, [c_vp, c_int, c_int, ctypes.POINTER(Pair), c_int, c_f64, c_i64, c_vp, c_vp, c_vp, c_vp, c_int, c_vp, c_vp]),
     "svx_concat_rows": (c_int, [c_vp, c_int, c_int, ctypes.POINTER(Pair), ctypes.POINTER(Frames), c_int, ctypes.POINTER(ConcatParams), c_i64,
                                 c_vp, c_vp, c_vp, c_vp, c_int, c_vp, c_vp]),
```

After: 9736 doc-pairs/s (median of 6 runs). About the same (+0.7%).
